# yangzhaojason/DualDiff

Measured on AMD Instinct MI355X. Metric: denoising-steps/sec, 6-view 224×400 fp16, 50-step DDIM @ 1/2/4/8 MI355X, higher is better.
Workload: dtype fp16; 1 GPU; BASELINE configs[1]: 6-view 224x400 (28x50 latents) multiview UNet + 2 ControlNet branches (ORS panorama + ORS-3D, SFA on), CFG 2.0 -> 12 view-instances/scene, DDIM-50 schedule, random-init weights; scenes_per_gpu=1, parallelism=scene-sharded x1 (no data-path collective), hip_graph=True, streams=3, invariant_conditioning=recomputed every step

## Files before the change

### dualdiff_amd/_native.py

```python
import ctypes
import os

import torch
from ctypes import (POINTER, Structure, c_char_p, c_float, c_int32, c_int64, c_uint32, c_void_p)

from . import _build

DD_F16, DD_BF16, DD_F32 = 0, 1, 2
DD_EPI_NONE, DD_EPI_GEGLU, DD_EPI_SILU = 0, 1, 2


class GemmDesc(Structure):
    _fields_ = [
        ("a", c_void_p), ("a2", c_void_p), ("lda", c_int64), ("lda2", c_int64), ("k1", c_int32),
        ("rows", c_int32), ("n", c_int32), ("k", c_int32),
        ("w", c_void_p), ("bias", c_void_p), ("rowvec", c_void_p),
        ("rows_per_inst", c_int32), ("ld_rowvec", c_int32),
        ("res", c_void_p), ("ldres", c_int64),
        ("out", c_void_p), ("ldc", c_int64),
        ("alpha", c_float), ("accumulate", c_int32), ("epilogue", c_int32),
        ("conv", c_int32), ("hin", c_int32), ("win", c_int32), ("cin", c_int32),
        ("hv", c_int32), ("wv", c_int32), ("hout", c_int32), ("wout", c_int32), ("stride", c_int32),
        ("dtype", c_int32), ("tile", c_int32), ("split_k", c_int32),
        ("ws", c_void_p), ("ws_bytes", c_int64),
        ("ln_colsum", c_void_p), ("ln_bias", c_void_p), ("ln_eps", c_float), ("out_f32", c_int32), ("ln_stats_out", c_void_p), ("ln_stats_in", c_void_p),
        ("out_headmajor_d", c_int32), ("hm_scaled_planes", c_int32), ("hm_scale", c_float),
        ("phase", c_int32),
        ("ln_out", c_void_p), ("ld_ln_out", c_int64), ("lno_gamma", c_void_p), ("lno_beta", c_void_p),
    ]


class AttnDesc(Structure):
    _fields_ = [
        ("q", c_void_p), ("k", c_void_p), ("v", c_void_p), ("o", c_void_p),
        ("ldq", c_int64), ("ldk", c_int64), ("ldv", c_int64), ("ldo", c_int64),
        ("q_batch_stride", c_int64), ("k_batch_stride", c_int64),
        ("v_batch_stride", c_int64), ("o_batch_stride", c_int64),
        ("batch", c_int32), ("heads", c_int32), ("head_dim", c_int32), ("lq", c_int32), ("lk", c_int32),
        ("scale", c_float),
        ("kv_batch_map", c_void_p),
        ("accumulate", c_int32), ("dtype", c_int32), ("variant", c_int32),
        ("q_head_stride", c_int64), ("k_head_stride", c_int64), ("v_head_stride", c_int64),
        ("q_prescaled", c_int32),
        ("kv_batch_map2", c_void_p),
        ("lk_dev", c_void_p),
    ]


class BoxTokensDesc(Structure):
    _fields_ = [
        ("points", c_void_p), ("classes", c_void_p), ("masks", c_void_p),
        ("class_tokens", c_void_p), ("null_pos", c_void_p), ("null_class", c_void_p),
        ("pos", c_void_p), ("cat", c_void_p), ("cls_out", c_void_p),
        ("rows", c_int32), ("points_per_box", c_int32), ("num_freqs", c_int32), ("include_input", c_int32),
        ("class_token_dim", c_int32), ("cls_offset", c_int32),
        ("ld_cat", c_int64),
        ("normalize", c_int32), ("points_dtype", c_int32), ("dtype", c_int32), ("n_classes", c_int32),
        ("freqs", c_float * 16), ("xyz_min", c_float * 3), ("xyz_range", c_float * 3),
    ]


class XAttnDesc(Structure):
    _fields_ = [
        ("x", c_void_p), ("ldx", c_int64), ("res", c_void_p), ("ldres", c_int64),
        ("wq", c_void_p), ("wo", c_void_p), ("bo", c_void_p),
        ("k", c_void_p), ("v", c_void_p), ("ldk", c_int64), ("ldv", c_int64),
        ("k_inst_stride", c_int64), ("k_head_stride", c_int64), ("v_inst_stride", c_int64), ("v_head_stride", c_int64),
        ("out", c_void_p), ("ldo", c_int64),
        ("instances", c_int32), ("rows_per_inst", c_int32), ("lk", c_int32),
        ("channels", c_int32), ("heads", c_int32), ("scale", c_float), ("dtype", c_int32),
        ("ln_out", c_void_p), ("ld_ln_out", c_int64), ("ln_gamma", c_void_p), ("ln_beta", c_void_p), ("ln_eps", c_float),
        ("lk_dev", c_void_p),
    ]


class Gemm8Desc(Structure):
    _fields_ = [
        ("a", c_void_p), ("a_scale", c_void_p), ("lda", c_int64),
        ("w", c_void_p), ("w_scale", c_void_p), ("ldw", c_int64),
        ("bias", c_void_p), ("res", c_void_p), ("ldres", c_int64),
        ("out", c_void_p), ("ldc", c_int64),
        ("rows", c_int32), ("n", c_int32), ("k_padded", c_int32), ("dtype", c_int32),
        ("out_headmajor_d", c_int32), ("hm_scaled_planes", c_int32), ("hm_scale", c_float), ("geglu", c_int32),
    ]


SIGNATURES = {
    "dd_abi_version": (c_int32, []),
    "dd_desc_size": (c_int64, [c_int32]),
    "dd_error_string": (c_char_p, [c_int32]),
    "dd_target_arch": (c_char_p, []),
    "dd_gemm": (c_int32, [POINTER(GemmDesc), c_void_p]),
    "dd_gemm_workspace_bytes": (c_int64, [POINTER(GemmDesc)]),
    "dd_gemm_num_tiles": (c_int32, []),
    "dd_gemm_tile_id": (c_int32, [c_int32]),
    "dd_gemm_kernel_name": (c_char_p, [POINTER(GemmDesc)]),
    "dd_gemm_conv_pad": (c_int32, [POINTER(GemmDesc), c_int32, c_void_p]),
    "dd_gemm_conv_pad_workspace_bytes": (c_int64, [POINTER(GemmDesc), c_int32]),
    "dd_gemm_conv_pad_kernel_name": (c_char_p, [POINTER(GemmDesc), c_int32]),
    "dd_groupnorm_nhwc": (c_int32, [c_void_p, c_int32, c_void_p, c_int32, c_void_p, c_void_p, c_void_p,
                                    c_int32, c_int32, c_int32, c_float, c_int32, c_int32,
                                    c_void_p, c_int64, c_void_p]),
    "dd_groupnorm_workspace_bytes": (c_int64, [c_int32, c_int32]),
    "dd_groupnorm_is_fused": (c_int32, [c_int32, c_int32, c_int32]),
    "dd_layernorm": (c_int32, [c_void_p, c_void_p, c_void_p, c_void_p, c_int64, c_int32, c_float,
                               c_int32, c_void_p]),
    "dd_attention": (c_int32, [POINTER(AttnDesc), c_void_p]),
    "dd_attention_kernel_name": (c_char_p, [POINTER(AttnDesc)]),
    "dd_add": (c_int32, [c_void_p, c_void_p, c_void_p, c_void_p, c_int64, c_int32, c_void_p]),
    "dd_scale": (c_int32, [c_void_p, c_void_p, c_float, c_int64, c_int32, c_void_p]),
    "dd_probe_spin": (c_int32, [c_void_p, c_uint32, c_void_p]),
    "dd_groupnorm_splitk": (c_int32, [c_void_p, c_int32, c_void_p, c_void_p, c_int32, c_void_p, c_int64, c_void_p,
                                      c_void_p, c_void_p, c_void_p, c_int32, c_int32, c_int32, c_int32, c_float, c_int32,
                                      c_int32, c_void_p]),
    "dd_xattn320": (c_int32, [POINTER(XAttnDesc), c_void_p]),
    "dd_nchw_to_nhwc_views": (c_int32, [c_void_p, c_void_p, c_int32, c_int32, c_int32, c_int32, c_int32, c_int32, c_int32,
                                        c_void_p]),
    "dd_fourier_embed_strided": (c_int32, [c_void_p, c_void_p, c_int64, c_int32, POINTER(c_float), c_int32, c_int32,
                                           c_int32, c_int32, c_int32, c_int64, c_int64, c_int64, c_int64, c_void_p]),
    "dd_box_tokens": (c_int32, [POINTER(BoxTokensDesc), c_void_p]),
    "dd_ctx_assemble": (c_int32, [c_void_p, c_void_p, c_void_p, c_void_p, c_void_p, c_int32, c_int32, c_int32, c_int32,
                                  c_int32, c_int32, c_int32, c_int32, c_void_p]),
    "dd_gemm8": (c_int32, [POINTER(Gemm8Desc), c_void_p]),
    "dd_rowquant_fp8": (c_int32, [c_void_p, c_void_p, c_void_p, c_void_p, c_void_p, c_int64, c_int32, c_int64, c_float,
                                  c_int32, c_void_p]),
    "dd_xattn_pack_weight": (c_int32, [c_void_p, c_void_p, c_int32, c_void_p]),
    "dd_silu": (c_int32, [c_void_p, c_void_p, c_int64, c_int32, c_void_p]),
    "dd_nchw_to_nhwc": (c_int32, [c_void_p, c_void_p, c_int32, c_int32, c_int32, c_int32, c_int32, c_void_p]),
    "dd_nhwc_to_nchw": (c_int32, [c_void_p, c_void_p, c_int32, c_int32, c_int32, c_int32, c_int32, c_void_p]),
    "dd_timestep_embedding": (c_int32, [c_void_p, c_void_p, c_int32, c_int32, c_int32, c_float,
                                        c_int32, c_void_p]),
    "dd_cfg_unipc_step": (c_int32, [c_void_p, c_void_p, c_void_p, c_void_p, c_void_p, c_void_p, c_void_p, c_void_p,
                                    c_float, c_int64, c_int32, c_void_p]),
    "dd_softmax_rows": (c_int32, [c_void_p, c_void_p, c_int64, c_int32, c_int64, c_int64, c_int32, c_void_p]),
    "dd_ors_project": (c_int32, [c_void_p, c_void_p, c_void_p, c_void_p, c_void_p, c_int32, c_int32, c_int32,
                                 c_float, c_int32, c_int32, c_int32, c_void_p]),
    "dd_fourier_embed": (c_int32, [c_void_p, c_void_p, c_int64, c_int32, POINTER(c_float), c_int32, c_int32,
                                   c_int32, c_int32, c_void_p]),
    "dd_conv3x3_small_cout": (c_int32, [c_void_p, c_void_p, c_void_p, c_void_p, c_int32, c_int32,
                                        c_int32, c_int32, c_int32, c_int32, c_void_p]),
    "dd_vae_posterior": (c_int32, [c_void_p, c_void_p, c_void_p, c_void_p, c_void_p, c_int32, c_int32, c_int32, c_float,
                                   c_int32, c_int32, c_void_p]),
    "dd_conv3x3_thin": (c_int32, [c_void_p, c_void_p, c_void_p, c_void_p, c_int32, c_int32, c_int32, c_int32, c_int32,
                                  c_int32, c_int32, c_int32, c_void_p]),
    "dd_cfg_ddim_step": (c_int32, [c_void_p, c_void_p, c_void_p, c_void_p, c_void_p, c_float,
                                   c_int64, c_int32, c_void_p]),
    "dd_cfg_ddim_step_given": (c_int32, [c_void_p, c_void_p, c_void_p, c_void_p, c_void_p, c_float, c_void_p, c_void_p,
                                         c_void_p, c_void_p, c_int32, c_int64, c_int64, c_int32, c_void_p]),
    "dd_cfg_unipc_step_given": (c_int32, [c_void_p, c_void_p, c_void_p, c_void_p, c_void_p, c_void_p, c_void_p,
                                          c_void_p, c_float, c_void_p, c_void_p, c_void_p, c_void_p, c_int32, c_int64,
                                          c_int64, c_int32, c_void_p]),
    "dd_given_views_noise": (c_int32, [c_void_p, c_void_p, c_void_p, c_void_p, c_void_p, c_float, c_float, c_int64,
                                       c_int64, c_int32, c_void_p]),
}

ABI_VERSION = 4
_LIB = None


def lib_path():
    return _build.lib_path()


def load(build_if_missing=True):
    global _LIB
    if _LIB is not None:
        return _LIB
    path = lib_path()
    if not os.path.exists(path):
        if not build_if_missing:
            raise RuntimeError("dualdiff_amd: %s is missing (run __graft_entry__.build())" % path)
        _build.build_native()
    try:
        lib = ctypes.CDLL(path)
    except OSError as e:
        raise RuntimeError("dualdiff_amd: cannot load HIP library %s: %s" % (path, e))
    for name, (res, args) in SIGNATURES.items():
        try:
            fn = getattr(lib, name)
        except AttributeError:
            raise RuntimeError("dualdiff_amd: %s does not export %s" % (path, name))
        fn.restype = res
        fn.argtypes = args
    if lib.dd_abi_version() != ABI_VERSION:
        raise RuntimeError("dualdiff_amd: %s has ABI version %d, this binding needs %d (rebuild: __graft_entry__.build())"
                           % (path, lib.dd_abi_version(), ABI_VERSION))
    for which, st in enumerate((GemmDesc, AttnDesc, XAttnDesc, Gemm8Desc, BoxTokensDesc)):
        if lib.dd_desc_size(which) != ctypes.sizeof(st):
            raise RuntimeError("dualdiff_amd: %s was built with a different %s (%d bytes, binding has %d)"
                               % (path, st.__name__, lib.dd_desc_size(which), ctypes.sizeof(st)))
    _LIB = lib
    return lib


class Unsupported(RuntimeError):
    """DD_ERR_UNSUPPORTED (-2): the library validated the call and launched NOTHING — the caller may take another form."""


def check(rc, what):
    if rc != 0:
        msg = load().dd_error_string(rc).decode()
        raise (Unsupported if rc == -2 else RuntimeError)("dualdiff_amd.%s failed: %s (%d)" % (what, msg, rc))
```

### dualdiff_amd/csrc/dd_debug.h

```cpp
#pragma once
#include <stdint.h>

namespace dd_dbg {
#ifdef DD_DBG_NODMA
constexpr bool NODMA = true;
#else
constexpr bool NODMA = false;
#endif
#ifdef DD_DBG_SAMEK
constexpr bool SAMEK = true;
#else
constexpr bool SAMEK = false;
#endif
#ifdef DD_DBG_NOLDS
constexpr bool NOLDS = true;
#else
constexpr bool NOLDS = false;
#endif
#ifdef DD_DBG_NOSECTOR
constexpr bool NOSECTOR = true;
#else
constexpr bool NOSECTOR = false;
#endif
#ifdef DD_DBG_C3_NODMA
constexpr bool C3_NODMA = true;
#else
constexpr bool C3_NODMA = false;
#endif
#ifdef DD_DBG_C3_NOWAIT
constexpr bool C3_NOWAIT = true;
#else
constexpr bool C3_NOWAIT = false;
#endif
#ifdef DD_DBG_C3_NOWREAD
constexpr bool C3_NOWREAD = true;
#else
constexpr bool C3_NOWREAD = false;
#endif
#ifdef DD_DBG_C3_NOGATHER
constexpr bool C3_NOGATHER = true;
#else
constexpr bool C3_NOGATHER = false;
#endif
#ifdef DD_DBG_NOSTAGE
constexpr bool NOSTAGE = true;
#else
constexpr bool NOSTAGE = false;
#endif
}

#ifdef DD_DBG_NOEXP
#define DD_EXP2(x) (x)
#else
#define DD_EXP2(x) __builtin_amdgcn_exp2f(x)
#endif

#ifndef DD_DBG_STORE_AUX
#define DD_DBG_STORE_AUX 0
#endif
#ifdef DD_DBG_NOSTORE
#define DD_G4_STORE_STATE() ((void)0)
#define DD_G4_STORE(...) ((void)0)
#elif defined(DD_DBG_ONESTORE)
#define DD_G4_STORE_STATE() bool g4_first = true
#define DD_G4_STORE(data, rsrc, voff, soff, aux) do { if (g4_first) __builtin_amdgcn_raw_buffer_store_b128(data, rsrc, voff, soff, 0); g4_first = false; } while (0)
#else
#define DD_G4_STORE_STATE() ((void)0)
#define DD_G4_STORE(data, rsrc, voff, soff, aux) __builtin_amdgcn_raw_buffer_store_b128(data, rsrc, voff, soff, DD_DBG_STORE_AUX)
#endif

#ifdef DD_DBG_C3_NOMFMA
#define C3_MFMA(w, x, a) ([&]() { asm volatile("" :: "v"(w), "v"(x)); return a; }())
#else
#define C3_MFMA(w, x, a) dd_mfma16(w, x, a)
#endif
#ifdef DD_DBG_C3_NOBAR
#define C3_BARRIER() ((void)0)
#else
#define C3_BARRIER() __builtin_amdgcn_s_barrier()
#endif

#ifdef DD_DBG_STAMP
#define DD_STAMP_DECL() uint64_t dbg_t[6]; const uint64_t dbg_r0 = __builtin_amdgcn_s_memrealtime()
#define DD_STAMP(i) do { if (threadIdx.x == 0) dbg_t[i] = __builtin_readcyclecounter(); } while (0)
#define DD_STAMP_IF(cond, i) do { if (cond) DD_STAMP(i); } while (0)
#define DD_STAMP_FLUSH(p)                                                                          \
  do {                                                                                             \
    DD_STAMP(5);                                                                                   \
    if (threadIdx.x == 0 && (p).dbg_stamps) {                                                      \
      uint64_t* o_ = (p).dbg_stamps + ((size_t)blockIdx.z * gridDim.x + blockIdx.x) * 8;          \
      for (int i_ = 0; i_ < 6; ++i_) o_[i_] = dbg_t[i_];                                           \
      o_[6] = dbg_r0;                                                                              \
      o_[7] = __builtin_amdgcn_s_memrealtime();                                                    \
    }                                                                                              \
  } while (0)
#define C3_SEG_DECL() uint64_t seg[5] = {0, 0, 0, 0, 0}; uint64_t seg_prev = 0
#define C3_SEG(k) do { const uint64_t now_ = __builtin_readcyclecounter(); if (s >= 9) seg[k] += now_ - seg_prev; seg_prev = now_; } while (0)
#define C3_SEG_FLUSH(p, wave, lane, nsteps)                                                                          \
  do {                                                                                                               \
    if (((wave) == 0 || (wave) == 4) && (lane) == 0 && (p).dbg_stamps) {                                             \
      uint64_t* o_ = (p).dbg_stamps + 65536 + (((size_t)blockIdx.z * gridDim.x + blockIdx.x) * 2 + ((wave) == 4)) * 8; \
      for (int i_ = 0; i_ < 5; ++i_) o_[i_] = seg[i_];                                                               \
      o_[5] = (nsteps) > 9 ? (nsteps) - 9 : 0;                                                                       \
      o_[6] = (wave);                                                                                                \
      o_[7] = 1;                                                                                                     \
    }                                                                                                                \
  } while (0)
#define DD_STAMP_HOST(p, d)                                                                                          \
  do {                                                                                                               \
    if ((d)->ws && (d)->ws_bytes >= (4 << 20))                                                                       \
      (p).dbg_stamps = reinterpret_cast<uint64_t*>(reinterpret_cast<char*>((d)->ws) + (d)->ws_bytes - (1 << 20));    \
  } while (0)
#else
#define DD_STAMP_DECL() ((void)0)
#define DD_STAMP(i) do {} while (0)
#define DD_STAMP_IF(cond, i) do {} while (0)
#define DD_STAMP_FLUSH(p) do {} while (0)
#define C3_SEG_DECL() ((void)0)
#define C3_SEG(k) do {} while (0)
#define C3_SEG_FLUSH(p, wave, lane, nsteps) do {} while (0)
#define DD_STAMP_HOST(p, d) do {} while (0)
#endif
```

### dualdiff_amd/csrc/norm.hip

```cpp
#include "dd_common.h"
#include <atomic>

namespace {

constexpr int GN_THREADS = 256;
constexpr int GN_MAX_SPLIT = 64;
constexpr int GN_MAX_C = 4096;

struct GnParams {
  const void* x1; const void* x2; int c1, c2, c;
  const void* gamma; const void* beta; void* y;
  int m, hw, groups, cpg; float eps; int silu;
  float* ws;
  int nsplit, pix_per_split;
  const float* sk_part; int sk_nsplit; int64_t sk_rows;
  const void* sk_bias; const void* sk_rowvec; int sk_ld_rowvec;
  const void* sk_res; int64_t sk_ldres;
  void* sk_xout;
};

struct GnMap { int cv_count, pl_count, cv, pl; bool active; };
__device__ __forceinline__ GnMap gn_map(int c) {
  GnMap mp;
  mp.cv_count = c >> 3;
  if (mp.cv_count >= GN_THREADS) {
    mp.pl_count = 1; mp.cv = threadIdx.x; mp.pl = 0; mp.active = true;
  } else {
    mp.pl_count = GN_THREADS / mp.cv_count;
    mp.cv = threadIdx.x % mp.cv_count;
    mp.pl = threadIdx.x / mp.cv_count;
    mp.active = mp.pl < mp.pl_count;
  }
  return mp;
}

template <typename T>
__device__ __forceinline__ const T* gn_src(const GnParams& p, int64_t row, int ch) {
  return ch < p.c1 ? reinterpret_cast<const T*>(p.x1) + row * p.c1 + ch
                   : reinterpret_cast<const T*>(p.x2) + row * p.c2 + (ch - p.c1);
}

constexpr int GN_UNROLL = 4;

template <typename T>
__device__ __forceinline__ float gn_pivot(const GnParams& p, int inst, int g) {
  return (float)*gn_src<T>(p, (int64_t)inst * p.hw, g * p.cpg);
}

template <typename T>
__device__ __forceinline__ u32x4 gn_sk_load8(const GnParams& p, int64_t row, int ch, int inst) {
  float v[8] = {0.f, 0.f, 0.f, 0.f, 0.f, 0.f, 0.f, 0.f};
  for (int z = 0; z < p.sk_nsplit; ++z) {
    const float* src = p.sk_part + ((int64_t)z * p.sk_rows + row) * p.c + ch;
    const f32x4 a = *reinterpret_cast<const f32x4*>(src);
    const f32x4 b = *reinterpret_cast<const f32x4*>(src + 4);
    v[0] += a[0]; v[1] += a[1]; v[2] += a[2]; v[3] += a[3];
    v[4] += b[0]; v[5] += b[1]; v[6] += b[2]; v[7] += b[3];
  }
  float b[8];
  if (p.sk_bias) {
    dd_unpack8<T>(dd_ld16(reinterpret_cast<const T*>(p.sk_bias) + ch), b);
#pragma unroll
    for (int i = 0; i < 8; ++i) v[i] += b[i];
  }
  if (p.sk_rowvec) {
    dd_unpack8<T>(dd_ld16(reinterpret_cast<const T*>(p.sk_rowvec) + (int64_t)inst * p.sk_ld_rowvec + ch), b);
#pragma unroll
    for (int i = 0; i < 8; ++i) v[i] += b[i];
  }
  if (p.sk_res) {
    dd_unpack8<T>(dd_ld16(reinterpret_cast<const T*>(p.sk_res) + row * p.sk_ldres + ch), b);
#pragma unroll
    for (int i = 0; i < 8; ++i) v[i] += b[i];
  }
  return dd_pack8<T>(v);
}

template <typename T>
__global__ __launch_bounds__(GN_THREADS)
void dd_gn_stats_kernel(const GnParams p) {
  __shared__ float s_a0[GN_THREADS], s_b0[GN_THREADS], s_a1[GN_THREADS], s_b1[GN_THREADS];
  __shared__ int s_g0[GN_THREADS], s_g1[GN_THREADS];
  const int split = blockIdx.x, inst = blockIdx.y;
  const GnMap mp = gn_map(p.c);
  const int p0 = split * p.pix_per_split;
  const int p1 = min(p.hw, p0 + p.pix_per_split);
  float gsum = 0.f, gsq = 0.f;
  for (int cv0 = 0; cv0 < mp.cv_count; cv0 += GN_THREADS) {
    const int cv = cv0 + mp.cv;
    int g0 = -1, g1 = -1;
    float a0 = 0.f, b0 = 0.f, a1 = 0.f, b1 = 0.f;
    if (mp.active && cv < mp.cv_count) {
      const int ch = cv << 3;
      float s[8], ss[8], pv[8];
      {
        const int ga = ch / p.cpg, gb = min((ch + 7) / p.cpg, p.groups - 1);
        const float pa = gn_pivot<T>(p, inst, ga), pb = gn_pivot<T>(p, inst, gb);
#pragma unroll
        for (int e = 0; e < 8; ++e) { s[e] = 0.f; ss[e] = 0.f; pv[e] = (ch + e) / p.cpg == ga ? pa : pb; }
      }
      int px = p0 + mp.pl;
      for (; px + (GN_UNROLL - 1) * mp.pl_count < p1; px += GN_UNROLL * mp.pl_count) {
        u32x4 v[GN_UNROLL];
#pragma unroll
        for (int u = 0; u < GN_UNROLL; ++u)
          v[u] = dd_ld16(gn_src<T>(p, (int64_t)inst * p.hw + px + u * mp.pl_count, ch));
#pragma unroll
        for (int u = 0; u < GN_UNROLL; ++u) {
          float f[8];
          dd_unpack8<T>(v[u], f);
#pragma unroll
          for (int e = 0; e < 8; ++e) { const float d = f[e] - pv[e]; s[e] += d; ss[e] += d * d; }
        }
      }
      for (; px < p1; px += mp.pl_count) {
        float f[8];
        dd_unpack8<T>(dd_ld16(gn_src<T>(p, (int64_t)inst * p.hw + px, ch)), f);
#pragma unroll
        for (int e = 0; e < 8; ++e) { const float d = f[e] - pv[e]; s[e] += d; ss[e] += d * d; }
      }
      g0 = ch / p.cpg;
      const int gl = (ch + 7) / p.cpg;
#pragma unroll
      for (int e = 0; e < 8; ++e) {
        const bool first = (ch + e) / p.cpg == g0;
        a0 += first ? s[e] : 0.f;  b0 += first ? ss[e] : 0.f;
        a1 += first ? 0.f : s[e];  b1 += first ? 0.f : ss[e];
      }
      g1 = gl != g0 ? gl : -1;
    }
    s_g0[threadIdx.x] = g0; s_a0[threadIdx.x] = a0; s_b0[threadIdx.x] = b0;
    s_g1[threadIdx.x] = g1; s_a1[threadIdx.x] = a1; s_b1[threadIdx.x] = b1;
    __syncthreads();
    if (threadIdx.x < p.groups) {
      const int g = threadIdx.x;
      const int lo = max((g * p.cpg) >> 3, cv0);
      const int hi = min(((g + 1) * p.cpg - 1) >> 3, min(cv0 + GN_THREADS, mp.cv_count) - 1);
      for (int pl = 0; pl < mp.pl_count; ++pl) {
        for (int c = lo; c <= hi; ++c) {
          const int t = mp.cv_count >= GN_THREADS ? (c - cv0) : pl * mp.cv_count + c;
          if (s_g0[t] == g) { gsum += s_a0[t]; gsq += s_b0[t]; }
          if (s_g1[t] == g) { gsum += s_a1[t]; gsq += s_b1[t]; }
        }
      }
    }
    __syncthreads();
  }
  if (threadIdx.x < p.groups) {
    float* dst = p.ws + (((int64_t)inst * p.nsplit + split) * p.groups + threadIdx.x) * 2;
    dst[0] = gsum;
    dst[1] = gsq;
  }
}

template <typename T>
__global__ __launch_bounds__(GN_THREADS)
void dd_gn_apply_kernel(const GnParams p) {
  __shared__ float s_mean[64], s_rstd[64];
  __shared__ float s_ps[GN_THREADS], s_pq[GN_THREADS];
  const int split = blockIdx.x, inst = blockIdx.y;
  const GnMap mp = gn_map(p.c);
  const int p0 = split * p.pix_per_split;
  const int p1 = min(p.hw, p0 + p.pix_per_split);
  const float my_pivot = (int)threadIdx.x < p.groups ? gn_pivot<T>(p, inst, threadIdx.x) : 0.f;
  const int cv_first = mp.cv;
  const int ch_first = min(cv_first, mp.cv_count - 1) << 3;
  u32x4 pre[GN_UNROLL];
  const bool pre_ok = mp.active && cv_first < mp.cv_count && p0 + mp.pl + (GN_UNROLL - 1) * mp.pl_count < p1;
  if (pre_ok) {
#pragma unroll
    for (int u = 0; u < GN_UNROLL; ++u)
      pre[u] = dd_ld16(gn_src<T>(p, (int64_t)inst * p.hw + p0 + mp.pl + u * mp.pl_count, ch_first));
  }
  {
    const int g = threadIdx.x % p.groups;
    const int chunk = threadIdx.x / p.groups;
    const int nchunk = GN_THREADS / p.groups;
    float s = 0.f, ss = 0.f;
    if (chunk < nchunk) {
      const float* src = p.ws + ((int64_t)inst * p.nsplit * p.groups + g) * 2;
      for (int i = chunk; i < p.nsplit; i += nchunk) {
        s += src[(int64_t)i * p.groups * 2];
        ss += src[(int64_t)i * p.groups * 2 + 1];
      }
    }
    s_ps[threadIdx.x] = s;
    s_pq[threadIdx.x] = ss;
    __syncthreads();
    if (threadIdx.x < p.groups) {
      float a = 0.f, b = 0.f;
      for (int c = 0; c < nchunk; ++c) { a += s_ps[c * p.groups + threadIdx.x]; b += s_pq[c * p.groups + threadIdx.x]; }
      const float inv_n = 1.0f / ((float)p.hw * (float)p.cpg);
      const float dm = a * inv_n;
      const float var = fmaxf(b * inv_n - dm * dm, 0.f);
      s_mean[threadIdx.x] = my_pivot + dm;
      s_rstd[threadIdx.x] = rsqrtf(var + p.eps);
    }
  }
  __syncthreads();
  if (!mp.active) return;
  for (int cv = mp.cv; cv < mp.cv_count; cv += GN_THREADS) {
    const int ch = cv << 3;
    float ga[8], be[8], sc[8], sh[8];
    dd_unpack8<T>(dd_ld16(reinterpret_cast<const T*>(p.gamma) + ch), ga);
    dd_unpack8<T>(dd_ld16(reinterpret_cast<const T*>(p.beta) + ch), be);
#pragma unroll
    for (int e = 0; e < 8; ++e) {
      const int g = (ch + e) / p.cpg;
      sc[e] = s_rstd[g] * ga[e];
      sh[e] = be[e] - s_mean[g] * sc[e];
    }
    auto apply_store = [&](u32x4 v, int64_t row) {
      float f[8];
      dd_unpack8<T>(v, f);
#pragma unroll
      for (int e = 0; e < 8; ++e) {
        const float y = f[e] * sc[e] + sh[e];
        f[e] = p.silu ? dd_silu_f(y) : y;
      }
      dd_st16(reinterpret_cast<T*>(p.y) + row * p.c + ch, dd_pack8<T>(f));
    };
    int px = p0 + mp.pl;
    if (cv == cv_first && pre_ok) {
#pragma unroll
      for (int u = 0; u < GN_UNROLL; ++u) apply_store(pre[u], (int64_t)inst * p.hw + px + u * mp.pl_count);
      px += GN_UNROLL * mp.pl_count;
    }
    for (; px + (GN_UNROLL - 1) * mp.pl_count < p1; px += GN_UNROLL * mp.pl_count) {
      u32x4 v[GN_UNROLL];
#pragma unroll
      for (int u = 0; u < GN_UNROLL; ++u)
        v[u] = dd_ld16(gn_src<T>(p, (int64_t)inst * p.hw + px + u * mp.pl_count, ch));
#pragma unroll
      for (int u = 0; u < GN_UNROLL; ++u) apply_store(v[u], (int64_t)inst * p.hw + px + u * mp.pl_count);
    }
    for (; px < p1; px += mp.pl_count)
      apply_store(dd_ld16(gn_src<T>(p, (int64_t)inst * p.hw + px, ch)), (int64_t)inst * p.hw + px);
  }
}


template <typename T, int THREADS, int NVMAX, bool SK = false>
__global__ __launch_bounds__(THREADS)
void dd_gn_fused_kernel(const GnParams p, int cpb, int vpp, int plc, int nv, int kred) {
  __shared__ float s_a0[THREADS], s_a1[THREADS], s_q0[THREADS], s_q1[THREADS];
  __shared__ float s_mean[64], s_rstd[64], s_piv[64];
  const int inst = blockIdx.y;
  const int t = threadIdx.x;
  const bool active = t < vpp * plc;
  const int cv = t % vpp, pl = t / vpp;
  const int gpb = cpb / p.cpg;
  const int lch = cv * 8;
  const int g0 = lch / p.cpg;
  const int g1 = min(g0 + 1, gpb - 1);
  const int nfirst = min(8, (g0 + 1) * p.cpg - lch);
  const int ch = blockIdx.x * cpb + min(cv, vpp - 1) * 8;
  u32x4 raw[NVMAX];
#pragma unroll
  for (int i = 0; i < NVMAX; ++i)
    if (i < nv) {
      const int64_t row = (int64_t)inst * p.hw + min(pl + i * plc, p.hw - 1);
      if constexpr (SK) {
        raw[i] = gn_sk_load8<T>(p, row, ch, inst);
        if (p.sk_xout && active && pl + i * plc < p.hw) dd_st16(reinterpret_cast<T*>(p.sk_xout) + row * p.c + ch, raw[i]);
      } else {
        raw[i] = dd_ld16(gn_src<T>(p, row, ch));
      }
    }
  const u32x4 graw = dd_ld16(reinterpret_cast<const T*>(p.gamma) + ch);
  const u32x4 braw = dd_ld16(reinterpret_cast<const T*>(p.beta) + ch);
  const float inv_n = 1.0f / ((float)p.hw * (float)p.cpg);

  float a0 = 0.f, a1 = 0.f, q0 = 0.f, q1 = 0.f;
  auto pivot = [&](int g) -> float {
    if constexpr (SK) {
      const int pc = g * p.cpg;
      float f[8];
      dd_unpack8<T>(gn_sk_load8<T>(p, (int64_t)inst * p.hw, pc & ~7, inst), f);
      float r = f[0];
#pragma unroll
      for (int e = 1; e < 8; ++e) r = (pc & 7) == e ? f[e] : r;
      return r;
    } else {
      return gn_pivot<T>(p, inst, g);
    }
  };
  const float piv0 = pivot(blockIdx.x * gpb + g0);
  const float piv1 = pivot(blockIdx.x * gpb + g1);
  if (t < gpb) s_piv[t] = pivot(blockIdx.x * gpb + t);
#pragma unroll
  for (int i = 0; i < NVMAX; ++i) {
    if (i < nv) {
      float f[8];
      dd_unpack8<T>(raw[i], f);
      const float keep = pl + i * plc < p.hw ? 1.f : 0.f;
#pragma unroll
      for (int e = 0; e < 8; ++e) {
        const float v = keep * (f[e] - (e < nfirst ? piv0 : piv1));
        if (e < nfirst) { a0 += v; q0 += v * v; } else { a1 += v; q1 += v * v; }
      }
    }
  }
  s_a0[t] = active ? a0 : 0.f; s_a1[t] = active ? a1 : 0.f;
  s_q0[t] = active ? q0 : 0.f; s_q1[t] = active ? q1 : 0.f;
  __syncthreads();
  {
    const int wave = t >> 6, lane = t & 63;
    for (int g = wave; g < gpb; g += THREADS / 64) {
      const int lo = (g * p.cpg) >> 3, hi = ((g + 1) * p.cpg - 1) >> 3;
      const int nvec = hi - lo + 1;
      const int n = plc * nvec;
      float sum = 0.f, sq = 0.f;
      for (int idx = lane; idx < n; idx += 64) {
        const int l = idx / nvec;
        const int c = lo + (idx - l * nvec);
        const int src = l * vpp + c;
        const int cg0 = (c * 8) / p.cpg;
        if (cg0 == g) { sum += s_a0[src]; sq += s_q0[src]; }
        else if (cg0 + 1 == g) { sum += s_a1[src]; sq += s_q1[src]; }
      }
      sum = dd_wave_sum(sum);
      sq = dd_wave_sum(sq);
      if (lane == 0) {
        const float dm = sum * inv_n;
        s_mean[g] = s_piv[g] + dm;
        s_rstd[g] = rsqrtf(fmaxf(sq * inv_n - dm * dm, 0.f) + p.eps);
      }
    }
  }
  __syncthreads();
  const float mean0 = s_mean[g0], mean1 = s_mean[g1];
  const float rstd0 = s_rstd[g0], rstd1 = s_rstd[g1];
  if (!active) return;
  float ga[8], be[8], sc[8], sh[8];
  dd_unpack8<T>(graw, ga);
  dd_unpack8<T>(braw, be);
#pragma unroll
  for (int e = 0; e < 8; ++e) {
    const float mu = e < nfirst ? mean0 : mean1, rs = e < nfirst ? rstd0 : rstd1;
    sc[e] = rs * ga[e];
    sh[e] = be[e] - mu * sc[e];
  }
#pragma unroll
  for (int i = 0; i < NVMAX; ++i) {
    const int px = pl + i * plc;
    if (i < nv && px < p.hw) {
      float f[8];
      dd_unpack8<T>(raw[i], f);
#pragma unroll
      for (int e = 0; e < 8; ++e) {
        const float y = f[e] * sc[e] + sh[e];
        f[e] = p.silu ? dd_silu_f(y) : y;
      }
      dd_st16(reinterpret_cast<T*>(p.y) + ((int64_t)inst * p.hw + px) * p.c + ch, dd_pack8<T>(f));
    }
  }
}

constexpr int GNF_NV_SMALL = 8;
constexpr int GNF_NV_BIG = 8;

bool gn_fused_plan(int hw, int c, int groups, int* cpb, int* vpp, int* plc, int* nv, int* kred, int* threads) {
  const int cpg = c / groups;
  for (int gpb = 1; gpb <= groups && gpb <= 64; ++gpb) {
    if (groups % gpb) continue;
    const int cb = cpg * gpb;
    if (cb % 8 || cb < 40) continue;
    const int v = cb / 8;
    static const int big_cap = getenv("DD_GN_BIG_CAP") ? atoi(getenv("DD_GN_BIG_CAP")) : 4;
    const int try_th[3] = {256, 1024, 256};
    const int try_cap[3] = {4, big_cap < GNF_NV_BIG ? big_cap : GNF_NV_BIG, GNF_NV_SMALL};
    for (int pass = 0; pass < 3; ++pass) {
      const int th = try_th[pass];
      if (v > th) continue;
      int pl = th / v;
      if (pl > hw) pl = hw;
      const int n = (hw + pl - 1) / pl;
      if (n > try_cap[pass]) continue;
      *cpb = cb; *vpp = v; *plc = pl; *nv = n; *kred = 0; *threads = th;
      return true;
    }
    return false;
  }
  return false;
}

constexpr int LN_MAXV = 4;

template <typename T>
__global__ __launch_bounds__(256)
void dd_layernorm_kernel(const T* __restrict__ x, const T* __restrict__ gamma,
                         const T* __restrict__ beta, T* __restrict__ y,
                         int64_t rows, int c, float eps) {
  const int lane = threadIdx.x & 63;
  const int64_t row = (int64_t)blockIdx.x * 4 + (threadIdx.x >> 6);
  if (row >= rows) return;
  const int nv = c >> 3;
  float f[LN_MAXV][8];
  float s = 0.f;
#pragma unroll
  for (int i = 0; i < LN_MAXV; ++i) {
    const int v = lane + i * 64;
    if (v < nv) {
      dd_unpack8<T>(dd_ld16(x + row * c + v * 8), f[i]);
#pragma unroll
      for (int e = 0; e < 8; ++e) s += f[i][e];
    }
  }
  const float mean = dd_wave_sum(s) / (float)c;
  float ss = 0.f;
#pragma unroll
  for (int i = 0; i < LN_MAXV; ++i) {
    const int v = lane + i * 64;
    if (v < nv) {
#pragma unroll
      for (int e = 0; e < 8; ++e) { const float d = f[i][e] - mean; ss += d * d; }
    }
  }
  const float rstd = rsqrtf(dd_wave_sum(ss) / (float)c + eps);
#pragma unroll
  for (int i = 0; i < LN_MAXV; ++i) {
    const int v = lane + i * 64;
    if (v < nv) {
      float ga[8], be[8], o[8];
      dd_unpack8<T>(dd_ld16(gamma + v * 8), ga);
      dd_unpack8<T>(dd_ld16(beta + v * 8), be);
#pragma unroll
      for (int e = 0; e < 8; ++e) o[e] = (f[i][e] - mean) * rstd * ga[e] + be[e];
      dd_st16(y + row * c + v * 8, dd_pack8<T>(o));
    }
  }
}

template <typename T, int LPR>
__global__ __launch_bounds__(256)
void dd_layernorm_sub_kernel(const T* __restrict__ x, const T* __restrict__ gamma,
                             const T* __restrict__ beta, T* __restrict__ y,
                             int64_t rows, float eps) {
  constexpr int VPL = 5;
  constexpr int C = LPR * VPL * 8;
  constexpr int RPW = 64 / LPR;
  const int lane = threadIdx.x & 63;
  const int sub = lane % LPR;
  const int64_t row = ((int64_t)blockIdx.x * 4 + (threadIdx.x >> 6)) * RPW + lane / LPR;
  const bool ok = row < rows;
  const int64_t r = ok ? row : rows - 1;
  u32x4 raw[VPL];
#pragma unroll
  for (int i = 0; i < VPL; ++i) raw[i] = dd_ld16(x + r * C + (sub + i * LPR) * 8);
  float f[VPL][8];
  float s = 0.f;
#pragma unroll
  for (int i = 0; i < VPL; ++i) {
    dd_unpack8<T>(raw[i], f[i]);
#pragma unroll
    for (int e = 0; e < 8; ++e) s += f[i][e];
  }
#pragma unroll
  for (int o = LPR / 2; o > 0; o >>= 1) s += __shfl_xor(s, o, 64);
  const float mean = s * (1.0f / (float)C);
  float ss = 0.f;
#pragma unroll
  for (int i = 0; i < VPL; ++i)
#pragma unroll
    for (int e = 0; e < 8; ++e) { const float d = f[i][e] - mean; ss += d * d; }
#pragma unroll
  for (int o = LPR / 2; o > 0; o >>= 1) ss += __shfl_xor(ss, o, 64);
  const float rstd = rsqrtf(ss * (1.0f / (float)C) + eps);
  if (!ok) return;
#pragma unroll
  for (int i = 0; i < VPL; ++i) {
    const int v = sub + i * LPR;
    float ga[8], be[8], o[8];
    dd_unpack8<T>(dd_ld16(gamma + v * 8), ga);
    dd_unpack8<T>(dd_ld16(beta + v * 8), be);
#pragma unroll
    for (int e = 0; e < 8; ++e) o[e] = (f[i][e] - mean) * rstd * ga[e] + be[e];
    dd_st16(y + row * C + v * 8, dd_pack8<T>(o));
  }
}

template <typename T>
bool launch_layernorm_sub(const void* x, const void* gamma, const void* beta, void* y, int64_t rows, int c,
                          float eps, hipStream_t s) {
  auto go = [&](auto kern, int lpr) {
    const int rpb = 4 * (64 / lpr);
    hipLaunchKernelGGL(kern, dim3((unsigned)((rows + rpb - 1) / rpb)), dim3(256), 0, s,
                       (const T*)x, (const T*)gamma, (const T*)beta, (T*)y, rows, eps);
  };
  switch (c) {
    case 320: go(dd_layernorm_sub_kernel<T, 8>, 8); return true;
    case 640: go(dd_layernorm_sub_kernel<T, 16>, 16); return true;
    case 1280: go(dd_layernorm_sub_kernel<T, 32>, 32); return true;
    default: return false;
  }
}

int gn_plan(int hw, int c, int* pix_per_split) {
  const int cv = c / 8;
  const int pl = cv >= GN_THREADS ? 1 : GN_THREADS / cv;
  int pps = (hw + GN_MAX_SPLIT - 1) / GN_MAX_SPLIT;
  const int min_pps = pl * GN_UNROLL;
  if (pps < min_pps) pps = min_pps;
  if (pps > hw) pps = hw;
  *pix_per_split = pps;
  return (hw + pps - 1) / pps;
}

}

extern "C" int64_t dd_groupnorm_workspace_bytes(int32_t m, int32_t groups) {
  if (m <= 0 || groups <= 0) return 0;
  return (int64_t)m * GN_MAX_SPLIT * groups * 2 * (int64_t)sizeof(float) + 256;
}

extern "C" int dd_groupnorm_nhwc(const void* x1, int32_t c1, const void* x2, int32_t c2,
                                 const void* gamma, const void* beta, void* y,
                                 int32_t m, int32_t hw, int32_t groups, float eps,
                                 int32_t apply_silu, int32_t dtype, void* ws, int64_t ws_bytes,
                                 dd_stream_t stream) {
  if (!x1 || !gamma || !beta || !y || !ws) return DD_ERR_BAD_ARG;
  if (c2 < 0 || (c2 > 0 && !x2)) return DD_ERR_BAD_ARG;
  const int c = c1 + c2;
  if (m <= 0 || hw <= 0 || groups <= 0 || groups > 64 || c1 <= 0) return DD_ERR_BAD_ARG;
  if ((c1 & 7) || (c2 & 7) || c % groups != 0 || c > GN_MAX_C) return DD_ERR_BAD_ARG;
  if (c / groups < 4) return DD_ERR_UNSUPPORTED;
  if (dtype != DD_F16 && dtype != DD_BF16) return DD_ERR_BAD_ARG;
  if (!dd_aligned16(x1) || (x2 && !dd_aligned16(x2)) || !dd_aligned16(y) ||
      !dd_aligned16(gamma) || !dd_aligned16(beta)) return DD_ERR_BAD_ARG;
  if (ws_bytes < dd_groupnorm_workspace_bytes(m, groups)) return DD_ERR_WORKSPACE;
  GnParams p{};
  p.x1 = x1; p.x2 = x2; p.c1 = c1; p.c2 = c2; p.c = c;
  p.gamma = gamma; p.beta = beta; p.y = y;
  p.m = m; p.hw = hw; p.groups = groups; p.cpg = c / groups; p.eps = eps; p.silu = apply_silu;
  p.ws = reinterpret_cast<float*>(ws) + 64;
  p.nsplit = gn_plan(hw, c, &p.pix_per_split);
  hipStream_t s = reinterpret_cast<hipStream_t>(stream);
  dd_clear_error();
  int cpb, vpp, plc, nv, kred, threads;
  if (gn_fused_plan(hw, c, groups, &cpb, &vpp, &plc, &nv, &kred, &threads)) {
    dim3 fgrid(c / cpb, m);
    if (threads == 256) {
      if (dtype == DD_F16) hipLaunchKernelGGL((dd_gn_fused_kernel<_Float16, 256, GNF_NV_SMALL>), fgrid, dim3(256), 0, s, p, cpb, vpp, plc, nv, kred);
      else hipLaunchKernelGGL((dd_gn_fused_kernel<__bf16, 256, GNF_NV_SMALL>), fgrid, dim3(256), 0, s, p, cpb, vpp, plc, nv, kred);
    } else {
      if (dtype == DD_F16) hipLaunchKernelGGL((dd_gn_fused_kernel<_Float16, 1024, GNF_NV_BIG>), fgrid, dim3(1024), 0, s, p, cpb, vpp, plc, nv, kred);
      else hipLaunchKernelGGL((dd_gn_fused_kernel<__bf16, 1024, GNF_NV_BIG>), fgrid, dim3(1024), 0, s, p, cpb, vpp, plc, nv, kred);
    }
    return dd_check_launch();
  }
  dim3 grid(p.nsplit, m);
  if (dtype == DD_F16) {
    hipLaunchKernelGGL(dd_gn_stats_kernel<_Float16>, grid, dim3(GN_THREADS), 0, s, p);
    hipLaunchKernelGGL(dd_gn_apply_kernel<_Float16>, grid, dim3(GN_THREADS), 0, s, p);
  } else {
    hipLaunchKernelGGL(dd_gn_stats_kernel<__bf16>, grid, dim3(GN_THREADS), 0, s, p);
    hipLaunchKernelGGL(dd_gn_apply_kernel<__bf16>, grid, dim3(GN_THREADS), 0, s, p);
  }
  return dd_check_launch();
}

extern "C" int dd_groupnorm_splitk(const float* partial, int32_t nsplit, const void* bias, const void* rowvec,
                                   int32_t ld_rowvec, const void* res, int64_t ldres, void* x_out,
                                   const void* gamma, const void* beta, void* y, int32_t m, int32_t hw, int32_t c,
                                   int32_t groups, float eps, int32_t apply_silu, int32_t dtype, dd_stream_t stream) {
  if (!partial || !gamma || !beta || !y || nsplit < 2 || nsplit > 64) return DD_ERR_BAD_ARG;
  if (m <= 0 || hw <= 0 || groups <= 0 || groups > 64 || c <= 0 || (c & 7) || c % groups || c > GN_MAX_C) return DD_ERR_BAD_ARG;
  if (c / groups < 4) return DD_ERR_UNSUPPORTED;
  if (dtype != DD_F16 && dtype != DD_BF16) return DD_ERR_BAD_ARG;
  if (!dd_aligned16(partial) || !dd_aligned16(y) || !dd_aligned16(gamma) || !dd_aligned16(beta) ||
      (bias && !dd_aligned16(bias)) || (rowvec && (!dd_aligned16(rowvec) || (ld_rowvec & 7))) ||
      (res && (!dd_aligned16(res) || (ldres & 7))) || (x_out && !dd_aligned16(x_out))) return DD_ERR_BAD_ARG;
  int cpb, vpp, plc, nv, kred, threads;
  if (!gn_fused_plan(hw, c, groups, &cpb, &vpp, &plc, &nv, &kred, &threads)) return DD_ERR_UNSUPPORTED;
  GnParams p{};
  p.x1 = nullptr; p.c1 = c; p.c = c;
  p.gamma = gamma; p.beta = beta; p.y = y;
  p.m = m; p.hw = hw; p.groups = groups; p.cpg = c / groups; p.eps = eps; p.silu = apply_silu;
  p.sk_part = partial; p.sk_nsplit = nsplit; p.sk_rows = (int64_t)m * hw;
  p.sk_bias = bias; p.sk_rowvec = rowvec; p.sk_ld_rowvec = ld_rowvec; p.sk_res = res; p.sk_ldres = ldres; p.sk_xout = x_out;
  hipStream_t s = reinterpret_cast<hipStream_t>(stream);
  dd_clear_error();
  dim3 fgrid(c / cpb, m);
  if (threads == 256) {
    if (dtype == DD_F16) hipLaunchKernelGGL((dd_gn_fused_kernel<_Float16, 256, GNF_NV_SMALL, true>), fgrid, dim3(256), 0, s, p, cpb, vpp, plc, nv, kred);
    else hipLaunchKernelGGL((dd_gn_fused_kernel<__bf16, 256, GNF_NV_SMALL, true>), fgrid, dim3(256), 0, s, p, cpb, vpp, plc, nv, kred);
  } else {
    if (dtype == DD_F16) hipLaunchKernelGGL((dd_gn_fused_kernel<_Float16, 1024, GNF_NV_BIG, true>), fgrid, dim3(1024), 0, s, p, cpb, vpp, plc, nv, kred);
    else hipLaunchKernelGGL((dd_gn_fused_kernel<__bf16, 1024, GNF_NV_BIG, true>), fgrid, dim3(1024), 0, s, p, cpb, vpp, plc, nv, kred);
  }
  return dd_check_launch();
}

extern "C" int dd_groupnorm_is_fused(int32_t hw, int32_t c, int32_t groups) {
  int cpb, vpp, plc, nv, kred, threads;
  if (hw <= 0 || c <= 0 || groups <= 0 || c % groups) return 0;
  return gn_fused_plan(hw, c, groups, &cpb, &vpp, &plc, &nv, &kred, &threads) ? threads : 0;
}

extern "C" int dd_layernorm(const void* x, const void* gamma, const void* beta, void* y,
                            int64_t rows, int32_t c, float eps, int32_t dtype,
                            dd_stream_t stream) {
  if (!x || !gamma || !beta || !y || rows <= 0 || c <= 0) return DD_ERR_BAD_ARG;
  if ((c & 7) || c > LN_MAXV * 512) return DD_ERR_UNSUPPORTED;
  if (dtype != DD_F16 && dtype != DD_BF16) return DD_ERR_BAD_ARG;
  if (!dd_aligned16(x) || !dd_aligned16(y) || !dd_aligned16(gamma) || !dd_aligned16(beta)) return DD_ERR_BAD_ARG;
  hipStream_t s = reinterpret_cast<hipStream_t>(stream);
  dd_clear_error();
  if (dtype == DD_F16 ? launch_layernorm_sub<_Float16>(x, gamma, beta, y, rows, c, eps, s)
                      : launch_layernorm_sub<__bf16>(x, gamma, beta, y, rows, c, eps, s))
    return dd_check_launch();
  const unsigned blocks = (unsigned)((rows + 3) / 4);
  if (dtype == DD_F16) {
    hipLaunchKernelGGL(dd_layernorm_kernel<_Float16>, dim3(blocks), dim3(256), 0, s,
                       (const _Float16*)x, (const _Float16*)gamma, (const _Float16*)beta,
                       (_Float16*)y, rows, c, eps);
  } else {
    hipLaunchKernelGGL(dd_layernorm_kernel<__bf16>, dim3(blocks), dim3(256), 0, s,
                       (const __bf16*)x, (const __bf16*)gamma, (const __bf16*)beta,
                       (__bf16*)y, rows, c, eps);
  }
  return dd_check_launch();
}
```

### include/dualdiff_hip.h

```cpp
#ifndef DUALDIFF_HIP_H
#define DUALDIFF_HIP_H

#include <stdint.h>

#ifdef __cplusplus
extern "C" {
#endif

#define DD_ABI_VERSION 4

enum { DD_F16 = 0, DD_BF16 = 1 };

enum {
  DD_OK = 0,
  DD_ERR_BAD_ARG = -1,
  DD_ERR_UNSUPPORTED = -2,
  DD_ERR_LAUNCH = -3,
  DD_ERR_WORKSPACE = -4
};

typedef void* dd_stream_t;

int dd_abi_version(void);
int64_t dd_desc_size(int which);
const char* dd_error_string(int code);
const char* dd_target_arch(void);

enum { DD_EPI_NONE = 0, DD_EPI_GEGLU = 1, DD_EPI_SILU = 2 };

typedef struct dd_gemm_desc {
  const void* a;
  const void* a2;
  int64_t lda, lda2;
  int32_t k1;
  int32_t rows, n, k;
  const void* w;
  const void* bias;
  const void* rowvec;
  int32_t rows_per_inst, ld_rowvec;
  const void* res;
  int64_t ldres;
  void* out;
  int64_t ldc;
  float alpha;
  int32_t accumulate;
  int32_t epilogue;
  int32_t conv;
  int32_t hin, win, cin;
  int32_t hv, wv;
  int32_t hout, wout, stride;
  int32_t dtype;
  int32_t tile;
  int32_t split_k;
  void* ws;
  int64_t ws_bytes;
  const void* ln_colsum;
  const void* ln_bias;
  float ln_eps;
  int32_t out_f32;
  void* ln_stats_out;
  const void* ln_stats_in;
  int32_t out_headmajor_d;
  int32_t hm_scaled_planes;
  float hm_scale;
  int32_t phase;
  void* ln_out;
  int64_t ld_ln_out;
  const void* lno_gamma;
  const void* lno_beta;
} dd_gemm_desc;

int dd_gemm(const dd_gemm_desc* d, dd_stream_t stream);
int64_t dd_gemm_workspace_bytes(const dd_gemm_desc* d);
int dd_gemm_num_tiles(void);
int dd_gemm_tile_id(int index);
const char* dd_gemm_kernel_name(const dd_gemm_desc* d);

int dd_gemm_conv_pad(const dd_gemm_desc* d, int32_t pad_lo, dd_stream_t stream);
int64_t dd_gemm_conv_pad_workspace_bytes(const dd_gemm_desc* d, int32_t pad_lo);
const char* dd_gemm_conv_pad_kernel_name(const dd_gemm_desc* d, int32_t pad_lo);

int dd_groupnorm_nhwc(const void* x1, int32_t c1, const void* x2, int32_t c2,
                      const void* gamma, const void* beta, void* y,
                      int32_t m, int32_t hw, int32_t groups, float eps,
                      int32_t apply_silu, int32_t dtype, void* ws, int64_t ws_bytes,
                      dd_stream_t stream);
int64_t dd_groupnorm_workspace_bytes(int32_t m, int32_t groups);
int dd_groupnorm_is_fused(int32_t hw, int32_t c, int32_t groups);
int dd_groupnorm_splitk(const float* partial, int32_t nsplit, const void* bias, const void* rowvec, int32_t ld_rowvec,
                        const void* res, int64_t ldres, void* x_out, const void* gamma, const void* beta, void* y,
                        int32_t m, int32_t hw, int32_t c, int32_t groups, float eps, int32_t apply_silu, int32_t dtype,
                        dd_stream_t stream);

int dd_layernorm(const void* x, const void* gamma, const void* beta, void* y,
                 int64_t rows, int32_t c, float eps, int32_t dtype, dd_stream_t stream);

typedef struct dd_attn_desc {
  const void* q; const void* k; const void* v; void* o;
  int64_t ldq, ldk, ldv, ldo;
  int64_t q_batch_stride, k_batch_stride, v_batch_stride, o_batch_stride;
  int32_t batch, heads, head_dim, lq, lk;
  float scale;
  const int32_t* kv_batch_map;
  int32_t accumulate;
  int32_t dtype;
  int32_t variant;
  int64_t q_head_stride, k_head_stride, v_head_stride;
  int32_t q_prescaled;
  const int32_t* kv_batch_map2;
  const int32_t* lk_dev;
} dd_attn_desc;

int dd_attention(const dd_attn_desc* d, dd_stream_t stream);
const char* dd_attention_kernel_name(const dd_attn_desc* d);

typedef struct dd_xattn_desc {
  const void* x; int64_t ldx;
  const void* res; int64_t ldres;
  const void* wq; const void* wo; const void* bo;
  const void* k; const void* v; int64_t ldk, ldv;
  int64_t k_inst_stride, k_head_stride, v_inst_stride, v_head_stride;
  void* out; int64_t ldo;
  int32_t instances, rows_per_inst, lk;
  int32_t channels, heads;
  float scale;
  int32_t dtype;
  void* ln_out; int64_t ld_ln_out;
  const void* ln_gamma; const void* ln_beta; float ln_eps;
  const int32_t* lk_dev;
} dd_xattn_desc;

int dd_xattn320(const dd_xattn_desc* d, dd_stream_t stream);
int dd_xattn_pack_weight(const void* w, void* packed, int32_t dtype, dd_stream_t stream);

int dd_add(const void* a, const void* b, const void* c, void* y, int64_t n,
           int32_t dtype, dd_stream_t stream);
int dd_scale(const void* x, void* y, float s, int64_t n, int32_t dtype, dd_stream_t stream);
int dd_silu(const void* x, void* y, int64_t n, int32_t dtype, dd_stream_t stream);

int dd_nchw_to_nhwc(const void* x, void* y, int32_t m, int32_t c, int32_t hw,
                    int32_t c_pad, int32_t dtype, dd_stream_t stream);
int dd_nhwc_to_nchw(const void* x, void* y, int32_t m, int32_t c, int32_t hw,
                    int32_t ldx, int32_t dtype, dd_stream_t stream);

int dd_timestep_embedding(const float* t, void* out, int32_t n, int32_t dim,
                          int32_t flip_sin_to_cos, float freq_shift,
                          int32_t dtype, dd_stream_t stream);

#define DD_F32 2
int dd_fourier_embed(const void* x, void* out, int64_t rows, int32_t dims, const float* freqs,
                     int32_t num_freqs, int32_t include_input, int32_t in_dtype, int32_t out_dtype,
                     dd_stream_t stream);

int dd_nchw_to_nhwc_views(const void* x, void* y, int32_t m, int32_t c, int32_t h, int32_t w, int32_t views,
                          int32_t c_pad, int32_t dtype, dd_stream_t stream);
int dd_fourier_embed_strided(const void* x, void* out, int64_t rows, int32_t dims, const float* freqs,
                             int32_t num_freqs, int32_t include_input, int32_t in_dtype, int32_t out_dtype,
                             int32_t inner, int64_t stride_outer, int64_t stride_inner, int64_t stride_dim,
                             int64_t out_ld, dd_stream_t stream);
typedef struct dd_box_tokens_desc {
  const void* points; const int64_t* classes; const uint8_t* masks;
  const void* class_tokens; const void* null_pos; const void* null_class;
  void* pos; void* cat; void* cls_out;
  int32_t rows, points_per_box, num_freqs, include_input, class_token_dim, cls_offset;
  int64_t ld_cat;
  int32_t normalize, points_dtype, dtype;
  int32_t n_classes;
  float freqs[16]; float xyz_min[3]; float xyz_range[3];
} dd_box_tokens_desc;
int dd_box_tokens(const dd_box_tokens_desc* d, dd_stream_t stream);
int dd_ctx_assemble(const void* cam, const void* text, const void* box, void* full, void* txt, int32_t m,
                    int32_t n_cam, int32_t lt, int32_t nbox, int32_t dim, int32_t text_per_view, int32_t box_views,
                    int32_t dtype, dd_stream_t stream);

int dd_ors_project(const uint8_t* occ, const float* origin, const float* dir, uint8_t* labels, void* cond,
                   int32_t n_cam, int32_t hw, int32_t samples, float step, int32_t keep_fg, int32_t keep_bg,
                   int32_t dtype, dd_stream_t stream);

int dd_softmax_rows(const float* s, void* p, int64_t rows, int32_t cols, int64_t lds, int64_t ldp,
                    int32_t dtype, dd_stream_t stream);

int dd_conv3x3_small_cout(const void* x, const void* w, const void* bias, void* y_nchw,
                          int32_t m, int32_t h, int32_t wd, int32_t cin, int32_t cout,
                          int32_t dtype, dd_stream_t stream);

int dd_vae_posterior(const void* moments, const float* wq, const float* bq, const void* noise, void* z,
                     int32_t m, int32_t h, int32_t w, float scale, int32_t out_f32, int32_t dtype, dd_stream_t stream);

int dd_conv3x3_thin(const void* x, const void* w, const void* bias, void* y, int32_t m, int32_t hin, int32_t win,
                    int32_t cin, int32_t cout, int32_t stride, int32_t silu, int32_t dtype, dd_stream_t stream);

int dd_cfg_ddim_step(const void* eps, const void* x, void* x_out, void* x_dup,
                     const float* coef, float guidance, int64_t n,
                     int32_t dtype, dd_stream_t stream);

int dd_cfg_unipc_step(const void* eps, const void* x, void* x_out, void* x_dup, float* last, float* m1,
                      float* m2, const float* coef, float guidance, int64_t n, int32_t dtype,
                      dd_stream_t stream);

int dd_cfg_ddim_step_given(const void* eps, const void* x, void* x_out, void* x_dup, const float* coef,
                           float guidance, const uint8_t* given, const float* clean, const void* noise0,
                           const float* gcoef, int32_t mode, int64_t n, int64_t view_elems, int32_t dtype,
                           dd_stream_t stream);
int dd_cfg_unipc_step_given(const void* eps, const void* x, void* x_out, void* x_dup, float* last, float* m1,
                            float* m2, const float* coef, float guidance, const uint8_t* given, const float* clean,
                            const void* noise0, const float* gcoef, int32_t mode, int64_t n, int64_t view_elems,
                            int32_t dtype, dd_stream_t stream);

int dd_given_views_noise(void* x, void* x_dup, const uint8_t* given, const float* clean, const void* noise0,
                         float sqrt_acp, float sqrt_1m_acp, int64_t n, int64_t view_elems, int32_t dtype,
                         dd_stream_t stream);

int dd_rowquant_fp8(const void* x, const void* gamma, const void* beta, void* q, float* scale, int64_t rows, int32_t c,
                    int64_t ldq, float eps, int32_t dtype, dd_stream_t stream);

typedef struct dd_gemm8_desc {
  const void* a; const float* a_scale; int64_t lda;
  const void* w; const float* w_scale; int64_t ldw;
  const void* bias; const void* res; int64_t ldres;
  void* out; int64_t ldc;
  int32_t rows, n, k_padded;
  int32_t dtype;
  int32_t out_headmajor_d, hm_scaled_planes; float hm_scale;
  int32_t geglu;
} dd_gemm8_desc;

int dd_gemm8(const dd_gemm8_desc* d, dd_stream_t stream);

int dd_probe_spin(uint64_t* stamps, uint32_t ticks_100mhz, dd_stream_t stream);

#ifdef __cplusplus
}
#endif
#endif
```

Measured before the change: 95.41 steps/s.

## Rework GroupNorm kernels: float reciprocal indexing, templated SiLU, wave-level reduction, adaptive split plan

Rewrites the GroupNorm stats, apply and fused kernels. Integer divisions are replaced by precomputed float reciprocals, and SiLU becomes a template parameter. The fused kernel's cross-thread reduction moves to per-wave float2 partials, and split-K pivots are read from already-loaded data instead of extra loads. The two-pass split planner now picks pixels-per-split to keep at least a minimum block count, and new debug switches plus a kernel-name query are added. Float-reciprocal division assumes exact rounding for small integers, and the larger reduction restructure risks correctness at edge shapes.

```diff
diff --git a/dualdiff_amd/_native.py b/dualdiff_amd/_native.py
--- a/dualdiff_amd/_native.py
+++ b/dualdiff_amd/_native.py
@@ -103,6 +103,7 @@
                                     c_void_p, c_int64, c_void_p]),
     "dd_groupnorm_workspace_bytes": (c_int64, [c_int32, c_int32]),
     "dd_groupnorm_is_fused": (c_int32, [c_int32, c_int32, c_int32]),
+    "dd_groupnorm_kernel_name": (c_char_p, [c_int32, c_int32, c_int32, c_int32, c_int32]),
     "dd_layernorm": (c_int32, [c_void_p, c_void_p, c_void_p, c_void_p, c_int64, c_int32, c_float,
                                c_int32, c_void_p]),
     "dd_attention": (c_int32, [POINTER(AttnDesc), c_void_p]),
diff --git a/dualdiff_amd/csrc/dd_debug.h b/dualdiff_amd/csrc/dd_debug.h
--- a/dualdiff_amd/csrc/dd_debug.h
+++ b/dualdiff_amd/csrc/dd_debug.h
@@ -46,6 +46,26 @@
 constexpr bool NOSTAGE = true;
 #else
 constexpr bool NOSTAGE = false;
+#endif
+#ifdef DD_DBG_GN_NORED
+constexpr bool GN_NORED = true;
+#else
+constexpr bool GN_NORED = false;
+#endif
+#ifdef DD_DBG_GN_NOSILU
+constexpr bool GN_NOSILU = true;
+#else
+constexpr bool GN_NOSILU = false;
+#endif
+#ifdef DD_DBG_GN_NOSTORE
+constexpr bool GN_NOSTORE = true;
+#else
+constexpr bool GN_NOSTORE = false;
+#endif
+#ifdef DD_DBG_GN_NOPIVOT
+constexpr bool GN_NOPIVOT = true;
+#else
+constexpr bool GN_NOPIVOT = false;
 #endif
 }
 
diff --git a/dualdiff_amd/csrc/norm.hip b/dualdiff_amd/csrc/norm.hip
--- a/dualdiff_amd/csrc/norm.hip
+++ b/dualdiff_amd/csrc/norm.hip
@@ -1,11 +1,16 @@
 #include "dd_common.h"
+#include "dd_debug.h"
 #include <atomic>
+#include <type_traits>
 
 namespace {
 
 constexpr int GN_THREADS = 256;
 constexpr int GN_MAX_SPLIT = 64;
 constexpr int GN_MAX_C = 4096;
+constexpr int GN_SMALL_NV = 4;
+constexpr int GN_FUSED_CAP = 4;
+constexpr int GN_MIN_BLOCKS = 512;
 
 struct GnParams {
   const void* x1; const void* x2; int c1, c2, c;
@@ -13,6 +18,7 @@
   int m, hw, groups, cpg; float eps; int silu;
   float* ws;
   int nsplit, pix_per_split;
+  float inv_cpg, inv_cvc, inv_groups; int pl_count, nchunk;
   const float* sk_part; int sk_nsplit; int64_t sk_rows;
   const void* sk_bias; const void* sk_rowvec; int sk_ld_rowvec;
   const void* sk_res; int64_t sk_ldres;
@@ -20,20 +26,6 @@
 };
 
 struct GnMap { int cv_count, pl_count, cv, pl; bool active; };
-__device__ __forceinline__ GnMap gn_map(int c) {
-  GnMap mp;
-  mp.cv_count = c >> 3;
-  if (mp.cv_count >= GN_THREADS) {
-    mp.pl_count = 1; mp.cv = threadIdx.x; mp.pl = 0; mp.active = true;
-  } else {
-    mp.pl_count = GN_THREADS / mp.cv_count;
-    mp.cv = threadIdx.x % mp.cv_count;
-    mp.pl = threadIdx.x / mp.cv_count;
-    mp.active = mp.pl < mp.pl_count;
-  }
-  return mp;
-}
-
 template <typename T>
 __device__ __forceinline__ const T* gn_src(const GnParams& p, int64_t row, int ch) {
   return ch < p.c1 ? reinterpret_cast<const T*>(p.x1) + row * p.c1 + ch
@@ -44,6 +36,7 @@
 
 template <typename T>
 __device__ __forceinline__ float gn_pivot(const GnParams& p, int inst, int g) {
+  if constexpr (dd_dbg::GN_NOPIVOT) return 0.f;
   return (float)*gn_src<T>(p, (int64_t)inst * p.hw, g * p.cpg);
 }
 
@@ -76,90 +69,104 @@
   return dd_pack8<T>(v);
 }
 
+__device__ __forceinline__ int gn_fdiv(int n, float inv) { return (int)(((float)n + 0.5f) * inv); }
+
+__device__ __forceinline__ GnMap gn_map2(const GnParams& p) {
+  GnMap mp;
+  mp.cv_count = p.c >> 3;
+  if (mp.cv_count >= GN_THREADS) {
+    mp.pl_count = 1; mp.cv = threadIdx.x; mp.pl = 0; mp.active = true;
+  } else {
+    mp.pl_count = p.pl_count;
+    mp.pl = gn_fdiv(threadIdx.x, p.inv_cvc);
+    mp.cv = threadIdx.x - mp.pl * mp.cv_count;
+    mp.active = mp.pl < mp.pl_count;
+  }
+  return mp;
+}
+
 template <typename T>
 __global__ __launch_bounds__(GN_THREADS)
 void dd_gn_stats_kernel(const GnParams p) {
   __shared__ float s_a0[GN_THREADS], s_b0[GN_THREADS], s_a1[GN_THREADS], s_b1[GN_THREADS];
-  __shared__ int s_g0[GN_THREADS], s_g1[GN_THREADS];
   const int split = blockIdx.x, inst = blockIdx.y;
-  const GnMap mp = gn_map(p.c);
+  const GnMap mp = gn_map2(p);
   const int p0 = split * p.pix_per_split;
   const int p1 = min(p.hw, p0 + p.pix_per_split);
   float gsum = 0.f, gsq = 0.f;
   for (int cv0 = 0; cv0 < mp.cv_count; cv0 += GN_THREADS) {
     const int cv = cv0 + mp.cv;
-    int g0 = -1, g1 = -1;
     float a0 = 0.f, b0 = 0.f, a1 = 0.f, b1 = 0.f;
     if (mp.active && cv < mp.cv_count) {
       const int ch = cv << 3;
+      const int ga = gn_fdiv(ch, p.inv_cpg), gb = min(ga + 1, p.groups - 1);
+      const int nfirst = min(8, (ga + 1) * p.cpg - ch);
+      const float pa = gn_pivot<T>(p, inst, ga), pb = gn_pivot<T>(p, inst, gb);
       float s[8], ss[8], pv[8];
-      {
-        const int ga = ch / p.cpg, gb = min((ch + 7) / p.cpg, p.groups - 1);
-        const float pa = gn_pivot<T>(p, inst, ga), pb = gn_pivot<T>(p, inst, gb);
-#pragma unroll
-        for (int e = 0; e < 8; ++e) { s[e] = 0.f; ss[e] = 0.f; pv[e] = (ch + e) / p.cpg == ga ? pa : pb; }
-      }
-      int px = p0 + mp.pl;
-      for (; px + (GN_UNROLL - 1) * mp.pl_count < p1; px += GN_UNROLL * mp.pl_count) {
-        u32x4 v[GN_UNROLL];
-#pragma unroll
-        for (int u = 0; u < GN_UNROLL; ++u)
-          v[u] = dd_ld16(gn_src<T>(p, (int64_t)inst * p.hw + px + u * mp.pl_count, ch));
-#pragma unroll
-        for (int u = 0; u < GN_UNROLL; ++u) {
+#pragma unroll
+      for (int e = 0; e < 8; ++e) { s[e] = 0.f; ss[e] = 0.f; pv[e] = e < nfirst ? pa : pb; }
+      auto batch = [&](auto U, int px) {
+        constexpr int N = decltype(U)::value;
+        u32x4 v[N];
+#pragma unroll
+        for (int u = 0; u < N; ++u) v[u] = dd_ld16(gn_src<T>(p, (int64_t)inst * p.hw + px + u * mp.pl_count, ch));
+#pragma unroll
+        for (int u = 0; u < N; ++u) {
           float f[8];
           dd_unpack8<T>(v[u], f);
 #pragma unroll
           for (int e = 0; e < 8; ++e) { const float d = f[e] - pv[e]; s[e] += d; ss[e] += d * d; }
         }
-      }
-      for (; px < p1; px += mp.pl_count) {
-        float f[8];
-        dd_unpack8<T>(dd_ld16(gn_src<T>(p, (int64_t)inst * p.hw + px, ch)), f);
-#pragma unroll
-        for (int e = 0; e < 8; ++e) { const float d = f[e] - pv[e]; s[e] += d; ss[e] += d * d; }
-      }
-      g0 = ch / p.cpg;
-      const int gl = (ch + 7) / p.cpg;
+      };
+      int px = p0 + mp.pl;
+      for (; px + (2 * GN_UNROLL - 1) * mp.pl_count < p1; px += 2 * GN_UNROLL * mp.pl_count) batch(std::integral_constant<int, 2 * GN_UNROLL>(), px);
+      for (; px + (GN_UNROLL - 1) * mp.pl_count < p1; px += GN_UNROLL * mp.pl_count) batch(std::integral_constant<int, GN_UNROLL>(), px);
+      for (; px < p1; px += mp.pl_count) batch(std::integral_constant<int, 1>(), px);
 #pragma unroll
       for (int e = 0; e < 8; ++e) {
-        const bool first = (ch + e) / p.cpg == g0;
+        const bool first = e < nfirst;
         a0 += first ? s[e] : 0.f;  b0 += first ? ss[e] : 0.f;
         a1 += first ? 0.f : s[e];  b1 += first ? 0.f : ss[e];
       }
-      g1 = gl != g0 ? gl : -1;
-    }
-    s_g0[threadIdx.x] = g0; s_a0[threadIdx.x] = a0; s_b0[threadIdx.x] = b0;
-    s_g1[threadIdx.x] = g1; s_a1[threadIdx.x] = a1; s_b1[threadIdx.x] = b1;
+    }
+    s_a0[threadIdx.x] = a0; s_b0[threadIdx.x] = b0; s_a1[threadIdx.x] = a1; s_b1[threadIdx.x] = b1;
     __syncthreads();
-    if (threadIdx.x < p.groups) {
+    if (!dd_dbg::GN_NORED && mp.pl_count > 1) {
+      if ((int)threadIdx.x < mp.cv_count) {
+        for (int pl = 1; pl < mp.pl_count; ++pl) {
+          const int src = pl * mp.cv_count + threadIdx.x;
+          a0 += s_a0[src]; b0 += s_b0[src]; a1 += s_a1[src]; b1 += s_b1[src];
+        }
+        s_a0[threadIdx.x] = a0; s_b0[threadIdx.x] = b0; s_a1[threadIdx.x] = a1; s_b1[threadIdx.x] = b1;
+      }
+      __syncthreads();
+    }
+    if (!dd_dbg::GN_NORED && (int)threadIdx.x < p.groups) {
       const int g = threadIdx.x;
       const int lo = max((g * p.cpg) >> 3, cv0);
       const int hi = min(((g + 1) * p.cpg - 1) >> 3, min(cv0 + GN_THREADS, mp.cv_count) - 1);
-      for (int pl = 0; pl < mp.pl_count; ++pl) {
-        for (int c = lo; c <= hi; ++c) {
-          const int t = mp.cv_count >= GN_THREADS ? (c - cv0) : pl * mp.cv_count + c;
-          if (s_g0[t] == g) { gsum += s_a0[t]; gsq += s_b0[t]; }
-          if (s_g1[t] == g) { gsum += s_a1[t]; gsq += s_b1[t]; }
-        }
+      for (int c = lo; c <= hi; ++c) {
+        const int cg0 = gn_fdiv(c << 3, p.inv_cpg);
+        if (cg0 == g) { gsum += s_a0[c - cv0]; gsq += s_b0[c - cv0]; }
+        else if (cg0 + 1 == g) { gsum += s_a1[c - cv0]; gsq += s_b1[c - cv0]; }
       }
     }
     __syncthreads();
   }
-  if (threadIdx.x < p.groups) {
+  if ((int)threadIdx.x < p.groups) {
     float* dst = p.ws + (((int64_t)inst * p.nsplit + split) * p.groups + threadIdx.x) * 2;
-    dst[0] = gsum;
-    dst[1] = gsq;
-  }
-}
-
-template <typename T>
+    dst[0] = dd_dbg::GN_NORED ? s_a0[threadIdx.x] : gsum;
+    dst[1] = dd_dbg::GN_NORED ? s_b0[threadIdx.x] : gsq;
+  }
+}
+
+template <typename T, bool SILU>
 __global__ __launch_bounds__(GN_THREADS)
 void dd_gn_apply_kernel(const GnParams p) {
   __shared__ float s_mean[64], s_rstd[64];
   __shared__ float s_ps[GN_THREADS], s_pq[GN_THREADS];
   const int split = blockIdx.x, inst = blockIdx.y;
-  const GnMap mp = gn_map(p.c);
+  const GnMap mp = gn_map2(p);
   const int p0 = split * p.pix_per_split;
   const int p1 = min(p.hw, p0 + p.pix_per_split);
   const float my_pivot = (int)threadIdx.x < p.groups ? gn_pivot<T>(p, inst, threadIdx.x) : 0.f;
@@ -173,23 +180,24 @@
       pre[u] = dd_ld16(gn_src<T>(p, (int64_t)inst * p.hw + p0 + mp.pl + u * mp.pl_count, ch_first));
   }
   {
-    const int g = threadIdx.x % p.groups;
-    const int chunk = threadIdx.x / p.groups;
-    const int nchunk = GN_THREADS / p.groups;
+    const int chunk = gn_fdiv(threadIdx.x, p.inv_groups);
+    const int g = threadIdx.x - chunk * p.groups;
+    const int nchunk = p.nchunk;
     float s = 0.f, ss = 0.f;
-    if (chunk < nchunk) {
-      const float* src = p.ws + ((int64_t)inst * p.nsplit * p.groups + g) * 2;
+    if (!dd_dbg::GN_NORED && chunk < nchunk) {
+      const float2* src = reinterpret_cast<const float2*>(p.ws) + (int64_t)inst * p.nsplit * p.groups + g;
       for (int i = chunk; i < p.nsplit; i += nchunk) {
-        s += src[(int64_t)i * p.groups * 2];
-        ss += src[(int64_t)i * p.groups * 2 + 1];
+        const float2 v = src[(int64_t)i * p.groups];
+        s += v.x;
+        ss += v.y;
       }
     }
     s_ps[threadIdx.x] = s;
     s_pq[threadIdx.x] = ss;
     __syncthreads();
-    if (threadIdx.x < p.groups) {
+    if ((int)threadIdx.x < p.groups) {
       float a = 0.f, b = 0.f;
-      for (int c = 0; c < nchunk; ++c) { a += s_ps[c * p.groups + threadIdx.x]; b += s_pq[c * p.groups + threadIdx.x]; }
+      for (int c = 0; c < (dd_dbg::GN_NORED ? 1 : nchunk); ++c) { a += s_ps[c * p.groups + threadIdx.x]; b += s_pq[c * p.groups + threadIdx.x]; }
       const float inv_n = 1.0f / ((float)p.hw * (float)p.cpg);
       const float dm = a * inv_n;
       const float var = fmaxf(b * inv_n - dm * dm, 0.f);
@@ -201,14 +209,16 @@
   if (!mp.active) return;
   for (int cv = mp.cv; cv < mp.cv_count; cv += GN_THREADS) {
     const int ch = cv << 3;
-    float ga[8], be[8], sc[8], sh[8];
-    dd_unpack8<T>(dd_ld16(reinterpret_cast<const T*>(p.gamma) + ch), ga);
-    dd_unpack8<T>(dd_ld16(reinterpret_cast<const T*>(p.beta) + ch), be);
+    const int ga = gn_fdiv(ch, p.inv_cpg), gb = min(ga + 1, p.groups - 1);
+    const int nfirst = min(8, (ga + 1) * p.cpg - ch);
+    const float mean_a = s_mean[ga], mean_b = s_mean[gb], rstd_a = s_rstd[ga], rstd_b = s_rstd[gb];
+    float ga8[8], be8[8], sc[8], sh[8];
+    dd_unpack8<T>(dd_ld16(reinterpret_cast<const T*>(p.gamma) + ch), ga8);
+    dd_unpack8<T>(dd_ld16(reinterpret_cast<const T*>(p.beta) + ch), be8);
 #pragma unroll
     for (int e = 0; e < 8; ++e) {
-      const int g = (ch + e) / p.cpg;
-      sc[e] = s_rstd[g] * ga[e];
-      sh[e] = be[e] - s_mean[g] * sc[e];
+      sc[e] = (e < nfirst ? rstd_a : rstd_b) * ga8[e];
+      sh[e] = be8[e] - (e < nfirst ? mean_a : mean_b) * sc[e];
     }
     auto apply_store = [&](u32x4 v, int64_t row) {
       float f[8];
@@ -216,9 +226,9 @@
 #pragma unroll
       for (int e = 0; e < 8; ++e) {
         const float y = f[e] * sc[e] + sh[e];
-        f[e] = p.silu ? dd_silu_f(y) : y;
-      }
-      dd_st16(reinterpret_cast<T*>(p.y) + row * p.c + ch, dd_pack8<T>(f));
+        f[e] = (SILU && !dd_dbg::GN_NOSILU) ? dd_silu_f(y) : y;
+      }
+      if (!dd_dbg::GN_NOSTORE || p.eps < 0.f) dd_st16(reinterpret_cast<T*>(p.y) + row * p.c + ch, dd_pack8<T>(f));
     };
     int px = p0 + mp.pl;
     if (cv == cv_first && pre_ok) {
@@ -240,29 +250,32 @@
 }
 
 
-template <typename T, int THREADS, int NVMAX, bool SK = false>
+constexpr int GN_GPB_MAX = 16;
+struct GnPlan { int cpb, vpp, plc, nv, gpb, threads; float inv_vpp; };
+
+template <typename T, int THREADS, int NVMAX, bool SILU, bool SK>
 __global__ __launch_bounds__(THREADS)
-void dd_gn_fused_kernel(const GnParams p, int cpb, int vpp, int plc, int nv, int kred) {
-  __shared__ float s_a0[THREADS], s_a1[THREADS], s_q0[THREADS], s_q1[THREADS];
-  __shared__ float s_mean[64], s_rstd[64], s_piv[64];
+void dd_gn_fused_kernel(const GnParams p, const GnPlan k) {
+  constexpr int NW = THREADS / 64;
+  __shared__ float2 s_part[NW][GN_GPB_MAX];
+  __shared__ float s_piv[GN_GPB_MAX];
   const int inst = blockIdx.y;
   const int t = threadIdx.x;
-  const bool active = t < vpp * plc;
-  const int cv = t % vpp, pl = t / vpp;
-  const int gpb = cpb / p.cpg;
+  const int pl = gn_fdiv(t, k.inv_vpp), cv = t - pl * k.vpp;
+  const bool active = pl < k.plc;
   const int lch = cv * 8;
-  const int g0 = lch / p.cpg;
-  const int g1 = min(g0 + 1, gpb - 1);
+  const int g0 = gn_fdiv(lch, p.inv_cpg);
+  const int g1 = min(g0 + 1, k.gpb - 1);
   const int nfirst = min(8, (g0 + 1) * p.cpg - lch);
-  const int ch = blockIdx.x * cpb + min(cv, vpp - 1) * 8;
+  const int ch = blockIdx.x * k.cpb + lch;
   u32x4 raw[NVMAX];
 #pragma unroll
   for (int i = 0; i < NVMAX; ++i)
-    if (i < nv) {
-      const int64_t row = (int64_t)inst * p.hw + min(pl + i * plc, p.hw - 1);
+    if (i < k.nv) {
+      const int64_t row = (int64_t)inst * p.hw + min(pl + i * k.plc, p.hw - 1);
       if constexpr (SK) {
         raw[i] = gn_sk_load8<T>(p, row, ch, inst);
-        if (p.sk_xout && active && pl + i * plc < p.hw) dd_st16(reinterpret_cast<T*>(p.sk_xout) + row * p.c + ch, raw[i]);
+        if (p.sk_xout && active && pl + i * k.plc < p.hw) dd_st16(reinterpret_cast<T*>(p.sk_xout) + row * p.c + ch, raw[i]);
       } else {
         raw[i] = dd_ld16(gn_src<T>(p, row, ch));
       }
@@ -271,29 +284,38 @@
   const u32x4 braw = dd_ld16(reinterpret_cast<const T*>(p.beta) + ch);
   const float inv_n = 1.0f / ((float)p.hw * (float)p.cpg);
 
+  float piv0 = 0.f, piv1 = 0.f;
+  if constexpr (SK) {
+    if constexpr (!dd_dbg::GN_NOPIVOT) {
+      if (pl == 0) {
+        float f[8];
+        dd_unpack8<T>(raw[0], f);
+#pragma unroll
+        for (int j = 0; j < 2; ++j) {
+          const int gl = g0 + j, off = gl * p.cpg - lch;
+          if (gl < k.gpb && off >= 0 && off < 8) {
+            float r = f[0];
+#pragma unroll
+            for (int e = 1; e < 8; ++e) r = off == e ? f[e] : r;
+            s_piv[gl] = r;
+          }
+        }
+      }
+      __syncthreads();
+      piv0 = s_piv[g0];
+      piv1 = s_piv[g1];
+    }
+  } else {
+    piv0 = gn_pivot<T>(p, inst, blockIdx.x * k.gpb + g0);
+    piv1 = gn_pivot<T>(p, inst, blockIdx.x * k.gpb + g1);
+  }
   float a0 = 0.f, a1 = 0.f, q0 = 0.f, q1 = 0.f;
-  auto pivot = [&](int g) -> float {
-    if constexpr (SK) {
-      const int pc = g * p.cpg;
-      float f[8];
-      dd_unpack8<T>(gn_sk_load8<T>(p, (int64_t)inst * p.hw, pc & ~7, inst), f);
-      float r = f[0];
-#pragma unroll
-      for (int e = 1; e < 8; ++e) r = (pc & 7) == e ? f[e] : r;
-      return r;
-    } else {
-      return gn_pivot<T>(p, inst, g);
-    }
-  };
-  const float piv0 = pivot(blockIdx.x * gpb + g0);
-  const float piv1 = pivot(blockIdx.x * gpb + g1);
-  if (t < gpb) s_piv[t] = pivot(blockIdx.x * gpb + t);
 #pragma unroll
   for (int i = 0; i < NVMAX; ++i) {
-    if (i < nv) {
+    if (i < k.nv) {
       float f[8];
       dd_unpack8<T>(raw[i], f);
-      const float keep = pl + i * plc < p.hw ? 1.f : 0.f;
+      const float keep = active && pl + i * k.plc < p.hw ? 1.f : 0.f;
 #pragma unroll
       for (int e = 0; e < 8; ++e) {
         const float v = keep * (f[e] - (e < nfirst ? piv0 : piv1));
@@ -301,37 +323,30 @@
       }
     }
   }
-  s_a0[t] = active ? a0 : 0.f; s_a1[t] = active ? a1 : 0.f;
-  s_q0[t] = active ? q0 : 0.f; s_q1[t] = active ? q1 : 0.f;
-  __syncthreads();
   {
     const int wave = t >> 6, lane = t & 63;
-    for (int g = wave; g < gpb; g += THREADS / 64) {
-      const int lo = (g * p.cpg) >> 3, hi = ((g + 1) * p.cpg - 1) >> 3;
-      const int nvec = hi - lo + 1;
-      const int n = plc * nvec;
-      float sum = 0.f, sq = 0.f;
-      for (int idx = lane; idx < n; idx += 64) {
-        const int l = idx / nvec;
-        const int c = lo + (idx - l * nvec);
-        const int src = l * vpp + c;
-        const int cg0 = (c * 8) / p.cpg;
-        if (cg0 == g) { sum += s_a0[src]; sq += s_q0[src]; }
-        else if (cg0 + 1 == g) { sum += s_a1[src]; sq += s_q1[src]; }
-      }
-      sum = dd_wave_sum(sum);
-      sq = dd_wave_sum(sq);
-      if (lane == 0) {
-        const float dm = sum * inv_n;
-        s_mean[g] = s_piv[g] + dm;
-        s_rstd[g] = rsqrtf(fmaxf(sq * inv_n - dm * dm, 0.f) + p.eps);
+    if constexpr (dd_dbg::GN_NORED) {
+      if (lane < k.gpb) s_part[wave][lane] = make_float2(a0 + a1, q0 + q1);
+    } else {
+      for (int g = 0; g < k.gpb; ++g) {
+        const float va = dd_wave_sum(g == g0 ? a0 : g == g1 ? a1 : 0.f);
+        const float vq = dd_wave_sum(g == g0 ? q0 : g == g1 ? q1 : 0.f);
+        if (lane == 0) s_part[wave][g] = make_float2(va, vq);
       }
     }
   }
   __syncthreads();
-  const float mean0 = s_mean[g0], mean1 = s_mean[g1];
-  const float rstd0 = s_rstd[g0], rstd1 = s_rstd[g1];
+  float sa0 = 0.f, sq0 = 0.f, sa1 = 0.f, sq1 = 0.f;
+#pragma unroll
+  for (int w = 0; w < NW; ++w) {
+    const float2 u0 = s_part[w][g0], u1 = s_part[w][g1];
+    sa0 += u0.x; sq0 += u0.y; sa1 += u1.x; sq1 += u1.y;
+  }
   if (!active) return;
+  const float dm0 = sa0 * inv_n, dm1 = sa1 * inv_n;
+  const float mean0 = piv0 + dm0, mean1 = piv1 + dm1;
+  const float rstd0 = rsqrtf(fmaxf(sq0 * inv_n - dm0 * dm0, 0.f) + p.eps);
+  const float rstd1 = rsqrtf(fmaxf(sq1 * inv_n - dm1 * dm1, 0.f) + p.eps);
   float ga[8], be[8], sc[8], sh[8];
   dd_unpack8<T>(graw, ga);
   dd_unpack8<T>(braw, be);
@@ -343,43 +358,53 @@
   }
 #pragma unroll
   for (int i = 0; i < NVMAX; ++i) {
-    const int px = pl + i * plc;
-    if (i < nv && px < p.hw) {
+    const int px = pl + i * k.plc;
+    if (i < k.nv && px < p.hw) {
       float f[8];
       dd_unpack8<T>(raw[i], f);
 #pragma unroll
       for (int e = 0; e < 8; ++e) {
         const float y = f[e] * sc[e] + sh[e];
-        f[e] = p.silu ? dd_silu_f(y) : y;
-      }
-      dd_st16(reinterpret_cast<T*>(p.y) + ((int64_t)inst * p.hw + px) * p.c + ch, dd_pack8<T>(f));
-    }
-  }
-}
-
-constexpr int GNF_NV_SMALL = 8;
-constexpr int GNF_NV_BIG = 8;
-
-bool gn_fused_plan(int hw, int c, int groups, int* cpb, int* vpp, int* plc, int* nv, int* kred, int* threads) {
+        f[e] = (SILU && !dd_dbg::GN_NOSILU) ? dd_silu_f(y) : y;
+      }
+      if (!dd_dbg::GN_NOSTORE || p.eps < 0.f)
+        dd_st16(reinterpret_cast<T*>(p.y) + ((int64_t)inst * p.hw + px) * p.c + ch, dd_pack8<T>(f));
+    }
+  }
+}
+
+constexpr int GNF_NV = 8;
+
+int gn_exp(const char* name) {
+  static const bool on = getenv("DD_GN_EXPERIMENT") != nullptr;
+  const char* v = on ? getenv(name) : nullptr;
+  return v ? atoi(v) : 0;
+}
+
+bool gn_fused_shape(int hw, int cpg, int cb, int th, GnPlan* k) {
+  const int v = cb / 8;
+  if (v > th) return false;
+  const int pl = th / v < hw ? th / v : hw;
+  const int n = (hw + pl - 1) / pl;
+  if (n > GNF_NV) return false;
+  k->cpb = cb; k->vpp = v; k->plc = pl; k->nv = n; k->gpb = cb / cpg; k->threads = th; k->inv_vpp = 1.0f / (float)v;
+  return true;
+}
+
+bool gn_fused_plan(int hw, int c, int groups, GnPlan* k) {
   const int cpg = c / groups;
-  for (int gpb = 1; gpb <= groups && gpb <= 64; ++gpb) {
+  static const int big_cap = getenv("DD_GN_BIG_CAP") ? atoi(getenv("DD_GN_BIG_CAP")) : GN_FUSED_CAP;
+  const int cmult = gn_exp("DD_GN_CMULT") > 0 ? gn_exp("DD_GN_CMULT") : 1;
+  for (int gpb = 1; gpb <= groups && gpb <= GN_GPB_MAX; ++gpb) {
     if (groups % gpb) continue;
-    const int cb = cpg * gpb;
+    int cb = cpg * gpb;
     if (cb % 8 || cb < 40) continue;
-    const int v = cb / 8;
-    static const int big_cap = getenv("DD_GN_BIG_CAP") ? atoi(getenv("DD_GN_BIG_CAP")) : 4;
-    const int try_th[3] = {256, 1024, 256};
-    const int try_cap[3] = {4, big_cap < GNF_NV_BIG ? big_cap : GNF_NV_BIG, GNF_NV_SMALL};
-    for (int pass = 0; pass < 3; ++pass) {
-      const int th = try_th[pass];
-      if (v > th) continue;
-      int pl = th / v;
-      if (pl > hw) pl = hw;
-      const int n = (hw + pl - 1) / pl;
-      if (n > try_cap[pass]) continue;
-      *cpb = cb; *vpp = v; *plc = pl; *nv = n; *kred = 0; *threads = th;
-      return true;
-    }
+    if (cmult > 1 && gpb * cmult <= GN_GPB_MAX && groups % (gpb * cmult) == 0) cb *= cmult;
+    const int forced = gn_exp("DD_GN_THREADS");
+    if (forced) return (forced == 256 || forced == 512 || forced == 1024) && gn_fused_shape(hw, cpg, cb, forced, k);
+    if (gn_fused_shape(hw, cpg, cb, 256, k) && k->nv <= GN_SMALL_NV) return true;
+    if (gn_fused_shape(hw, cpg, cb, 512, k) && k->nv <= GN_SMALL_NV) return true;
+    if (gn_fused_shape(hw, cpg, cb, 1024, k) && k->nv <= (big_cap < GNF_NV ? big_cap : GNF_NV)) return true;
     return false;
   }
   return false;
@@ -496,15 +521,52 @@
   }
 }
 
-int gn_plan(int hw, int c, int* pix_per_split) {
+int gn_plan(int m, int hw, int c, int* pix_per_split) {
   const int cv = c / 8;
   const int pl = cv >= GN_THREADS ? 1 : GN_THREADS / cv;
-  int pps = (hw + GN_MAX_SPLIT - 1) / GN_MAX_SPLIT;
-  const int min_pps = pl * GN_UNROLL;
-  if (pps < min_pps) pps = min_pps;
+  const int floor_pps = (hw + GN_MAX_SPLIT - 1) / GN_MAX_SPLIT;
+  int mult = gn_exp("DD_GN_PPS_MULT");
+  if (mult <= 0) {
+    mult = 4;
+    while (mult > 1 && (int64_t)((hw + pl * GN_UNROLL * mult - 1) / (pl * GN_UNROLL * mult)) * m < GN_MIN_BLOCKS) --mult;
+  }
+  int pps = pl * GN_UNROLL * mult;
+  if (pps < floor_pps) pps = (floor_pps + pl - 1) / pl * pl;
   if (pps > hw) pps = hw;
   *pix_per_split = pps;
   return (hw + pps - 1) / pps;
+}
+
+void gn_fill(GnParams& p, int m, int hw, int c, int groups, float eps, int silu) {
+  p.c = c; p.m = m; p.hw = hw; p.groups = groups; p.cpg = c / groups; p.eps = eps; p.silu = silu;
+  p.inv_cpg = 1.0f / (float)p.cpg;
+  p.inv_cvc = 1.0f / (float)(c / 8);
+  p.inv_groups = 1.0f / (float)groups;
+  p.pl_count = c / 8 >= GN_THREADS ? 1 : GN_THREADS / (c / 8);
+  p.nchunk = GN_THREADS / groups;
+}
+
+template <typename T, bool SK>
+void gn_launch_fused_t(const GnParams& p, const GnPlan& k, hipStream_t s) {
+  const dim3 grid(p.c / k.cpb, p.m);
+  auto go = [&](auto kern) { hipLaunchKernelGGL(kern, grid, dim3(k.threads), 0, s, p, k); };
+  if (p.silu) {
+    if (k.threads == 256) go(dd_gn_fused_kernel<T, 256, GNF_NV, true, SK>);
+    else if (k.threads == 512) go(dd_gn_fused_kernel<T, 512, GNF_NV, true, SK>);
+    else go(dd_gn_fused_kernel<T, 1024, GNF_NV, true, SK>);
+  } else {
+    if (k.threads == 256) go(dd_gn_fused_kernel<T, 256, GNF_NV, false, SK>);
+    else if (k.threads == 512) go(dd_gn_fused_kernel<T, 512, GNF_NV, false, SK>);
+    else go(dd_gn_fused_kernel<T, 1024, GNF_NV, false, SK>);
+  }
+}
+
+template <typename T>
+void gn_launch_two(const GnParams& p, hipStream_t s) {
+  const dim3 grid(p.nsplit, p.m);
+  hipLaunchKernelGGL(dd_gn_stats_kernel<T>, grid, dim3(GN_THREADS), 0, s, p);
+  if (p.silu) hipLaunchKernelGGL((dd_gn_apply_kernel<T, true>), grid, dim3(GN_THREADS), 0, s, p);
+  else hipLaunchKernelGGL((dd_gn_apply_kernel<T, false>), grid, dim3(GN_THREADS), 0, s, p);
 }
 
 }
@@ -530,33 +592,21 @@
       !dd_aligned16(gamma) || !dd_aligned16(beta)) return DD_ERR_BAD_ARG;
   if (ws_bytes < dd_groupnorm_workspace_bytes(m, groups)) return DD_ERR_WORKSPACE;
   GnParams p{};
-  p.x1 = x1; p.x2 = x2; p.c1 = c1; p.c2 = c2; p.c = c;
+  p.x1 = x1; p.x2 = x2; p.c1 = c1; p.c2 = c2;
   p.gamma = gamma; p.beta = beta; p.y = y;
-  p.m = m; p.hw = hw; p.groups = groups; p.cpg = c / groups; p.eps = eps; p.silu = apply_silu;
+  gn_fill(p, m, hw, c, groups, eps, apply_silu);
   p.ws = reinterpret_cast<float*>(ws) + 64;
-  p.nsplit = gn_plan(hw, c, &p.pix_per_split);
   hipStream_t s = reinterpret_cast<hipStream_t>(stream);
   dd_clear_error();
-  int cpb, vpp, plc, nv, kred, threads;
-  if (gn_fused_plan(hw, c, groups, &cpb, &vpp, &plc, &nv, &kred, &threads)) {
-    dim3 fgrid(c / cpb, m);
-    if (threads == 256) {
-      if (dtype == DD_F16) hipLaunchKernelGGL((dd_gn_fused_kernel<_Float16, 256, GNF_NV_SMALL>), fgrid, dim3(256), 0, s, p, cpb, vpp, plc, nv, kred);
-      else hipLaunchKernelGGL((dd_gn_fused_kernel<__bf16, 256, GNF_NV_SMALL>), fgrid, dim3(256), 0, s, p, cpb, vpp, plc, nv, kred);
-    } else {
-      if (dtype == DD_F16) hipLaunchKernelGGL((dd_gn_fused_kernel<_Float16, 1024, GNF_NV_BIG>), fgrid, dim3(1024), 0, s, p, cpb, vpp, plc, nv, kred);
-      else hipLaunchKernelGGL((dd_gn_fused_kernel<__bf16, 1024, GNF_NV_BIG>), fgrid, dim3(1024), 0, s, p, cpb, vpp, plc, nv, kred);
-    }
+  GnPlan k;
+  if (gn_fused_plan(hw, c, groups, &k)) {
+    if (dtype == DD_F16) gn_launch_fused_t<_Float16, false>(p, k, s);
+    else gn_launch_fused_t<__bf16, false>(p, k, s);
     return dd_check_launch();
   }
-  dim3 grid(p.nsplit, m);
-  if (dtype == DD_F16) {
-    hipLaunchKernelGGL(dd_gn_stats_kernel<_Float16>, grid, dim3(GN_THREADS), 0, s, p);
-    hipLaunchKernelGGL(dd_gn_apply_kernel<_Float16>, grid, dim3(GN_THREADS), 0, s, p);
-  } else {
-    hipLaunchKernelGGL(dd_gn_stats_kernel<__bf16>, grid, dim3(GN_THREADS), 0, s, p);
-    hipLaunchKernelGGL(dd_gn_apply_kernel<__bf16>, grid, dim3(GN_THREADS), 0, s, p);
-  }
+  p.nsplit = gn_plan(m, hw, c, &p.pix_per_split);
+  if (dtype == DD_F16) gn_launch_two<_Float16>(p, s);
+  else gn_launch_two<__bf16>(p, s);
   return dd_check_launch();
 }
 
@@ -571,31 +621,43 @@
   if (!dd_aligned16(partial) || !dd_aligned16(y) || !dd_aligned16(gamma) || !dd_aligned16(beta) ||
       (bias && !dd_aligned16(bias)) || (rowvec && (!dd_aligned16(rowvec) || (ld_rowvec & 7))) ||
       (res && (!dd_aligned16(res) || (ldres & 7))) || (x_out && !dd_aligned16(x_out))) return DD_ERR_BAD_ARG;
-  int cpb, vpp, plc, nv, kred, threads;
-  if (!gn_fused_plan(hw, c, groups, &cpb, &vpp, &plc, &nv, &kred, &threads)) return DD_ERR_UNSUPPORTED;
+  GnPlan k;
+  if (!gn_fused_plan(hw, c, groups, &k)) return DD_ERR_UNSUPPORTED;
   GnParams p{};
-  p.x1 = nullptr; p.c1 = c; p.c = c;
+  p.x1 = nullptr; p.c1 = c;
   p.gamma = gamma; p.beta = beta; p.y = y;
-  p.m = m; p.hw = hw; p.groups = groups; p.cpg = c / groups; p.eps = eps; p.silu = apply_silu;
+  gn_fill(p, m, hw, c, groups, eps, apply_silu);
   p.sk_part = partial; p.sk_nsplit = nsplit; p.sk_rows = (int64_t)m * hw;
   p.sk_bias = bias; p.sk_rowvec = rowvec; p.sk_ld_rowvec = ld_rowvec; p.sk_res = res; p.sk_ldres = ldres; p.sk_xout = x_out;
   hipStream_t s = reinterpret_cast<hipStream_t>(stream);
   dd_clear_error();
-  dim3 fgrid(c / cpb, m);
-  if (threads == 256) {
-    if (dtype == DD_F16) hipLaunchKernelGGL((dd_gn_fused_kernel<_Float16, 256, GNF_NV_SMALL, true>), fgrid, dim3(256), 0, s, p, cpb, vpp, plc, nv, kred);
-    else hipLaunchKernelGGL((dd_gn_fused_kernel<__bf16, 256, GNF_NV_SMALL, true>), fgrid, dim3(256), 0, s, p, cpb, vpp, plc, nv, kred);
+  if (dtype == DD_F16) gn_launch_fused_t<_Float16, true>(p, k, s);
+  else gn_launch_fused_t<__bf16, true>(p, k, s);
+  return dd_check_launch();
+}
+
+extern "C" int dd_groupnorm_is_fused(int32_t hw, int32_t c, int32_t groups) {
+  GnPlan k;
+  if (hw <= 0 || c <= 0 || groups <= 0 || c % groups) return 0;
+  return gn_fused_plan(hw, c, groups, &k) ? k.threads : 0;
+}
+
+extern "C" const char* dd_groupnorm_kernel_name(int32_t m, int32_t hw, int32_t c, int32_t groups, int32_t dtype) {
+  thread_local char name[192];
+  if (m <= 0 || hw <= 0 || groups <= 0 || groups > 64 || c <= 0 || (c & 7) || c % groups != 0 || c > GN_MAX_C) return "invalid";
+  if (dtype != DD_F16 && dtype != DD_BF16) return "invalid";
+  if (c / groups < 4) return "unsupported";
+  const char* tn = dtype == DD_F16 ? "f16" : "bf16";
+  GnPlan k;
+  if (gn_fused_plan(hw, c, groups, &k)) {
+    snprintf(name, sizeof(name), "dd_gn_fused_kernel<%s, %d, %d> cpb=%d vpp=%d plc=%d nv=%d grid=%dx%d",
+             tn, k.threads, GNF_NV, k.cpb, k.vpp, k.plc, k.nv, c / k.cpb, m);
   } else {
-    if (dtype == DD_F16) hipLaunchKernelGGL((dd_gn_fused_kernel<_Float16, 1024, GNF_NV_BIG, true>), fgrid, dim3(1024), 0, s, p, cpb, vpp, plc, nv, kred);
-    else hipLaunchKernelGGL((dd_gn_fused_kernel<__bf16, 1024, GNF_NV_BIG, true>), fgrid, dim3(1024), 0, s, p, cpb, vpp, plc, nv, kred);
-  }
-  return dd_check_launch();
-}
-
-extern "C" int dd_groupnorm_is_fused(int32_t hw, int32_t c, int32_t groups) {
-  int cpb, vpp, plc, nv, kred, threads;
-  if (hw <= 0 || c <= 0 || groups <= 0 || c % groups) return 0;
-  return gn_fused_plan(hw, c, groups, &cpb, &vpp, &plc, &nv, &kred, &threads) ? threads : 0;
+    int pps;
+    const int ns = gn_plan(m, hw, c, &pps);
+    snprintf(name, sizeof(name), "dd_gn_stats_kernel<%s> + dd_gn_apply_kernel<%s> nsplit=%d pps=%d grid=%dx%d", tn, tn, ns, pps, ns, m);
+  }
+  return name;
 }
 
 extern "C" int dd_layernorm(const void* x, const void* gamma, const void* beta, void* y,
diff --git a/include/dualdiff_hip.h b/include/dualdiff_hip.h
--- a/include/dualdiff_hip.h
+++ b/include/dualdiff_hip.h
@@ -87,6 +87,7 @@
                       dd_stream_t stream);
 int64_t dd_groupnorm_workspace_bytes(int32_t m, int32_t groups);
 int dd_groupnorm_is_fused(int32_t hw, int32_t c, int32_t groups);
+const char* dd_groupnorm_kernel_name(int32_t m, int32_t hw, int32_t c, int32_t groups, int32_t dtype);
 int dd_groupnorm_splitk(const float* partial, int32_t nsplit, const void* bias, const void* rowvec, int32_t ld_rowvec,
                         const void* res, int64_t ldres, void* x_out, const void* gamma, const void* beta, void* y,
                         int32_t m, int32_t hw, int32_t c, int32_t groups, float eps, int32_t apply_silu, int32_t dtype,
```

After: 96.30 steps/s (median of 6 runs). About the same (+0.9%).
